# pablode/gatling

Hardware: AMD Instinct MI355X
Metric: Msamples/s (spp x pixels / s) at 8 bounces, 1920x1080 (higher is better)
Workload: dtype f32; 1 GPU; C2: cornell.usda 1920x1080 spp=1024 max-bounces=8 UsdPreviewSurface (diffuse + GGX specular), NEE off; width=1920, height=1080, spp=1024, max_bounces=8, parallelism=single, triangles=46, bvh8_nodes=4

## Files before the change

### gatling_amd/capi.py

```python
from __future__ import annotations

import ctypes as C
import os

import numpy as np

from .scene import P_COUNT, SceneDesc, RenderSettings

_HERE = os.path.dirname(os.path.abspath(__file__))
LIB_PATH = os.path.join(_HERE, "libgatling_gi.so")
if os.environ.get("GATLING_GI_LIB"):
    LIB_PATH = os.path.abspath(os.environ["GATLING_GI_LIB"])

GI_C_OK = 0
AOV_COLOR = 0
FORMAT_INT32, FORMAT_FLOAT32, FORMAT_FLOAT32_VEC4 = 0, 1, 2
OPTION_COUNT_TRAVERSAL, OPTION_KERNEL_TIMERS, OPTION_POOL_SLOTS, OPTION_SAMPLE_BUFFER_MB, OPTION_TRACE_DYNAMIC, OPTION_TWO_LEVEL, OPTION_FUSED_PATH, OPTION_DEVICES = 1, 2, 3, 4, 5, 6, 7, 8
OPTION_SAMPLE_LOOKAHEAD = 10
OPTION_VERTEX_UPDATES = 12
OPTION_VISIBILITY_UPDATES = 11
OPTION_TOPOLOGY_UPDATES = 13
OPTION_RESYNC_REFITS = 14
OPTION_BVH_BUILD = 9

# ... 57 lines not shown
    _fields_ = [("texture", C.c_void_p), ("wrapS", C.c_int32), ("wrapT", C.c_int32), ("channel", C.c_int32),
                ("scale", C.c_float * 4), ("bias", C.c_float * 4)]


class GiCPrimvarData(C.Structure):
    _fields_ = [("name", C.c_char_p), ("type", C.c_int32), ("interpolation", C.c_int32), ("data", C.c_void_p), ("dataSize", C.c_uint64)]



ASSET_OPEN = C.CFUNCTYPE(C.c_void_p, C.c_void_p, C.c_char_p)
ASSET_SIZE = C.CFUNCTYPE(C.c_uint64, C.c_void_p, C.c_void_p)
ASSET_DATA = C.CFUNCTYPE(C.c_void_p, C.c_void_p, C.c_void_p)
ASSET_CLOSE = C.CFUNCTYPE(None, C.c_void_p, C.c_void_p)


class GiCAssetReader(C.Structure):
    _fields_ = [("user", C.c_void_p), ("open", ASSET_OPEN), ("size", ASSET_SIZE), ("data", ASSET_DATA), ("close", ASSET_CLOSE)]


class GiCDecodedImage(C.Structure):
    _fields_ = [("format", C.c_uint32), ("width", C.c_uint32), ("height", C.c_uint32), ("reserved", C.c_uint32), ("pixels", C.c_void_p), ("handle", C.c_void_p)]


IMAGE_LOAD = C.CFUNCTYPE(C.c_int32, C.c_void_p, C.c_char_p, C.c_void_p, C.c_uint64, C.c_int32, C.POINTER(GiCDecodedImage))
IMAGE_RELEASE = C.CFUNCTYPE(None, C.c_void_p, C.POINTER(GiCDecodedImage))
IMAGE_RGBA8_UNORM, IMAGE_RGB16_FLOAT, IMAGE_RGBA16_FLOAT, IMAGE_R32_FLOAT, IMAGE_RGBA32_FLOAT = 1, 2, 3, 4, 5


class GiCImageLoader(C.Structure):
    _fields_ = [("user", C.c_void_p), ("load", IMAGE_LOAD), ("release", IMAGE_RELEASE)]


SYMBOLS = [
    ("giCInitialize", C.c_int, [C.c_int]), ("giCInitializeDevices", C.c_int, [C.POINTER(C.c_int32), C.c_uint32]), ("giCGetDeviceCount", C.c_uint32, []), ("giCGetApiVersion", C.c_uint32, []), ("giCGetDevicePeerAccess", C.c_int32, [C.c_uint32]), ("giCTerminate", None, []), ("giCGetLastError", C.c_char_p, []),
    ("giCCreateMaterial", _P, [_P, C.c_char_p, C.POINTER(GiCMaterialDesc)]), ("giCDestroyMaterial", None, [_P]),
    ("giCCreateMesh", _P, [_P, C.POINTER(GiCMeshDesc)]), ("giCSetMeshTransform", None, [_P, _FP]),
    ("giCSetMeshInstanceTransforms", None, [_P, _U, _FP]), ("giCSetMeshInstanceIds", None, [_P, _U, C.POINTER(C.c_int32)]),
    ("giCSetMeshMaterial", None, [_P, _P]), ("giCSetMeshVisibility", None, [_P, _I]), ("giCSetMeshVertices", C.c_int, [_P, _U, _P]), ("giCDestroyMesh", None, [_P]),
    ("giCRender", C.c_int, [C.POINTER(GiCRenderParams)]),
    ("giCCreateScene", _P, []), ("giCDestroyScene", None, [_P]),
    ("giCCreateSphereLight", _P, [_P]), ("giCDestroySphereLight", None, [_P, _P]), ("giCSetSphereLightPosition", None, [_P, _FP]),
    ("giCSetSphereLightBaseEmission", None, [_P, _FP]), ("giCSetSphereLightRadius", None, [_P, _F, _F, _F]),
    ("giCSetSphereLightDiffuseSpecular", None, [_P, _F, _F]),
    ("giCCreateDistantLight", _P, [_P]), ("giCDestroyDistantLight", None, [_P, _P]), ("giCSetDistantLightDirection", None, [_P, _FP]),
    ("giCSetDistantLightBaseEmission", None, [_P, _FP]), ("giCSetDistantLightAngle", None, [_P, _F]),
    ("giCSetDistantLightDiffuseSpecular", None, [_P, _F, _F]),
    ("giCCreateRectLight", _P, [_P]), ("giCDestroyRectLight", None, [_P, _P]), ("giCSetRectLightOrigin", None, [_P, _FP]),
    ("giCSetRectLightTangents", None, [_P, _FP, _FP]), ("giCSetRectLightBaseEmission", None, [_P, _FP]),
    ("giCSetRectLightDimensions", None, [_P, _F, _F]), ("giCSetRectLightDiffuseSpecular", None, [_P, _F, _F]),
    ("giCCreateDiskLight", _P, [_P]), ("giCDestroyDiskLight", None, [_P, _P]), ("giCSetDiskLightOrigin", None, [_P, _FP]),
    ("giCSetDiskLightTangents", None, [_P, _FP, _FP]), ("giCSetDiskLightBaseEmission", None, [_P, _FP]),
    ("giCSetDiskLightRadius", None, [_P, _F, _F]), ("giCSetDiskLightDiffuseSpecular", None, [_P, _F, _F]),
    ("giCCreateDomeLight", _P, [_P, C.c_char_p]), ("giCDestroyDomeLight", None, [_P]), ("giCSetDomeLightRotation", None, [_P, _FP]),
    ("giCSetDomeLightBaseEmission", None, [_P, _FP]), ("giCSetDomeLightDiffuseSpecular", None, [_P, _F, _F]),
    ("giCSetDomeLightTexture", None, [_P, _P]),
    ("giCCreateTexture", _P, [_P, C.POINTER(GiCTextureDesc)]), ("giCDestroyTexture", None, [_P]),
    ("giCCreateTextureFromFile", _P, [_P, C.c_char_p, _I]),
    ("giCDebugDecodeImage", C.c_int, [C.c_char_p, _I, C.POINTER(C.c_uint32), C.POINTER(C.c_uint32), _FP, C.c_uint64]),
    ("giCRegisterAssetReader", None, [C.POINTER(GiCAssetReader)]), ("giCSetImageLoader", None, [C.POINTER(GiCImageLoader)]),
    ("giCSetMaterialTexture", C.c_int, [_P, _I, C.POINTER(GiCTextureBinding)]),
    ("giCSetMaterialTextureTransform", C.c_int, [_P, _I, _FP]),
    ("giCSetMeshPrimvars", C.c_int, [_P, _U, C.POINTER(GiCPrimvarData)]), ("giCSetMeshInstancerPrimvars", C.c_int, [_P, _U, C.POINTER(GiCPrimvarData)]),
    ("giCSetMaterialPrimvarInput", C.c_int, [_P, _I, C.c_char_p]),
    ("giCCreateRenderBuffer", _P, [_U, _U, _I]), ("giCDestroyRenderBuffer", None, [_P]), ("giCGetRenderBufferMem", _P, [_P]),
    ("giCGetRenderBufferDeviceMem", _P, [_P]), ("giCSetRenderBufferDeviceOnly", None, [_P, _I]),
    ("giCGetRenderStats", C.c_int, [_P, C.POINTER(GiCRenderStats)]), ("giCSetSceneOption", C.c_int, [_P, _I, _I]),
    ("giCGetLookaheadStats", C.c_int, [_P, C.POINTER(GiCLookaheadStats)]),
    ("giCTraceRays", C.c_int, [_P, _U, _FP, _FP, _F, _F, _FP, C.POINTER(C.c_int32)]),
    ("giCDebugEvalBsdf", C.c_int, [C.POINTER(GiCMaterialDesc), _U, _FP, _FP]),
    ("giCDebugShadeClass", C.c_int, [C.POINTER(GiCMaterialDesc)]),
    ("giCDebugCheckSqrt", C.c_int64, [C.c_uint32, C.c_uint64]),
    ("giCDebugValidateBvh", C.c_int, [_FP, _U, C.POINTER(C.c_uint32), C.POINTER(C.c_uint32)]),
    ("giCDebugValidatePartitionedBvh", C.c_int, [_FP, _U, _U, C.POINTER(C.c_uint32), C.POINTER(C.c_uint32)]),
    ("giCDebugValidateSceneBvh", C.c_int, [_P, _U, C.POINTER(C.c_uint32), C.POINTER(C.c_uint32), C.POINTER(C.c_int32), C.POINTER(C.c_uint64)]),
    ("giCDebugTexRuntime", C.c_int, [_FP, _U, _U, _U, _U, _FP, _FP]),
    ("giCDebugEditDirtyFlags", C.c_int32, [_I, _I]), ("giCDebugSceneUpdateCounts", C.c_int, [_P, C.POINTER(C.c_uint64)]),
    ("giCDebugSceneVisibilityUpdateCount", C.c_int, [_P, C.POINTER(C.c_uint64)]), ("giCDebugSceneClassState", C.c_int, [_P, C.POINTER(C.c_uint32)]),
    ("giCDebugSceneVertexUpdateCount", C.c_int, [_P, C.POINTER(C.c_uint64)]), ("giCDebugRefitBvh", C.c_int, [_FP, _FP, _U, C.POINTER(C.c_uint32), C.POINTER(C.c_uint32)]),
    ("giCDebugSceneRefitCheck", C.c_int, [_P, _U, C.POINTER(C.c_uint32)]),
    ("giCDebugSceneTopologyUpdateCount", C.c_int, [_P, C.POINTER(C.c_uint64)]),
    ("giCDebugSceneResyncCount", C.c_int, [_P, C.POINTER(C.c_uint64)]), ("giCDebugGatherShade", C.c_int, [_P, _U, _P, _U]),
    ("giCDebugSceneShadeCheck", C.c_int, [_P, _U, C.POINTER(C.c_uint32)]),
    ("giCDebugPathWalkStats", C.c_int, [_P, C.POINTER(C.c_uint64)]),
    ("giCDebugMissRect", C.c_int, [_FP, C.POINTER(GiCCameraDesc), C.POINTER(GiCRenderSettings), _U, _U, C.POINTER(C.c_uint32)]),
]

_lib = None


def load_library():
    global _lib
    if _lib is None:
        if not os.path.exists(LIB_PATH):
            raise RuntimeError(f"{LIB_PATH} is missing: build it with `python -c 'import __graft_entry__ as g; g.build()'` "
                               "(hipcc --offload-arch=gfx950); there is no CPU fallback")
        L = C.CDLL(LIB_PATH)
        for name, res, args in SYMBOLS:
            fn = getattr(L, name)
            fn.restype = res
            fn.argtypes = args
        _lib = L
    return _lib


def _fp(values):
    arr = (C.c_float * len(values))(*[float(v) for v in values])
    return arr


class GiError(RuntimeError):
    pass


def miss_rect(bounds, camera, rs: "RenderSettings", width: int, height: int):
    L = load_library()
    out = (C.c_uint32 * 4)()
    cam, st = _camera(camera), _settings(rs)
    if L.giCDebugMissRect(_fp(bounds), C.byref(cam), C.byref(st), int(width), int(height), out) != GI_C_OK:
        raise GiError("giCDebugMissRect failed: " + L.giCGetLastError().decode())
    return tuple(int(v) for v in out)


def debug_gather_shade(vertices, faces) -> int:
    from .scene import VERTEX_DTYPE
    L = load_library()
    v = np.ascontiguousarray(vertices, VERTEX_DTYPE)
    f = np.ascontiguousarray(faces, np.uint32).reshape(-1, 3)
    n = L.giCDebugGatherShade(v.ctypes.data, len(v), f.ctypes.data, len(f))
    if n < 0:
        raise GiError("giCDebugGatherShade refused the mesh")
    return int(n)


_initialized = False


def initialize(device: int = 0, devices=None):
    global _initialized
    L = load_library()
    if not _initialized:
        if devices:
            arr = (C.c_int32 * len(devices))(*[int(d) for d in devices])
            rc = L.giCInitializeDevices(arr, len(devices))
        else:
            rc = L.giCInitialize(device)
        if rc != GI_C_OK:
            raise GiError("giCInitialize failed: " + L.giCGetLastError().decode())
        _initialized = True
    return L


def _camera(cam) -> GiCCameraDesc:
    f3 = lambda v: (C.c_float * 3)(*[float(x) for x in v])
    return GiCCameraDesc(f3(cam.position), f3(cam.forward), f3(cam.up), cam.vfov, cam.f_stop, cam.focus_distance,
                         cam.focal_length, cam.clip_start, cam.clip_end, cam.exposure)


def _settings(rs: RenderSettings) -> GiCRenderSettings:
    s = GiCRenderSettings()
    s.clippingPlanes = int(rs.clipping_planes); s.depthOfField = int(rs.depth_of_field)
    s.domeLightCameraVisible = int(rs.dome_light_camera_visible); s.filterImportanceSampling = int(rs.filter_importance_sampling)
    s.frame = float(getattr(rs, "frame", 0.0)); s.jitteredSampling = int(rs.jittered_sampling); s.lightIntensityMultiplier = rs.light_intensity_multiplier
    s.maxBounces = rs.max_bounces; s.maxSampleValue = rs.max_sample_value; s.maxVolumeWalkLength = rs.max_volume_walk_length
    s.mediumStackSize = rs.medium_stack_size; s.metersPerSceneUnit = rs.meters_per_scene_unit
    s.nextEventEstimation = int(rs.next_event_estimation); s.progressiveAccumulation = int(rs.progressive_accumulation)
    s.rrBounceOffset = rs.rr_bounce_offset; s.rrInvMinTermProb = rs.rr_inv_min_term_prob; s.spp = rs.spp; s.time = 0.0
# ... 181 lines not shown
        else:
            m.primvar_inputs.pop(slot, None)
        if self.L.giCSetMaterialPrimvarInput(self.materials[material_index], int(slot), name.encode() if name else None) != GI_C_OK:
            raise GiError("giCSetMaterialPrimvarInput failed: " + self.L.giCGetLastError().decode())

    def _set_primvars(self, fn, h, pvs):
        arr, keep = (GiCPrimvarData * max(len(pvs), 1))(), []
        for k, pv in enumerate(pvs):
            d = np.ascontiguousarray(pv.data, np.int32 if int(pv.type) >= 4 else np.float32).reshape(-1)
            keep.append(d)
            arr[k] = GiCPrimvarData(pv.name.encode(), int(pv.type), int(pv.interpolation), d.ctypes.data, d.nbytes)
        if fn(h, len(pvs), arr) != GI_C_OK:
            raise GiError("giCSetMesh*Primvars failed: " + self.L.giCGetLastError().decode())

    def set_mesh_primvars(self, mesh_index: int, primvars):
        self.desc.meshes[mesh_index].primvars = list(primvars)
        self._set_primvars(self.L.giCSetMeshPrimvars, self.meshes[mesh_index], list(primvars))

    def set_mesh_instancer_primvars(self, mesh_index: int, primvars):
        self.desc.meshes[mesh_index].instancer_primvars = list(primvars)
        self._set_primvars(self.L.giCSetMeshInstancerPrimvars, self.meshes[mesh_index], list(primvars))

    def set_mesh_visibility(self, mesh_index: int, visible: bool):
        self.desc.meshes[mesh_index].visible = bool(visible)
        self.L.giCSetMeshVisibility(self.meshes[mesh_index], int(bool(visible)))

    def set_mesh_vertices(self, mesh_index: int, vertices):
        from .scene import VERTEX_DTYPE
        v = np.ascontiguousarray(vertices, VERTEX_DTYPE)
        if self.L.giCSetMeshVertices(self.meshes[mesh_index], len(v), v.ctypes.data) != GI_C_OK:
            raise GiError("giCSetMeshVertices failed: " + self.L.giCGetLastError().decode())
        self.desc.meshes[mesh_index].vertices = v.copy()

    def vertex_update_count(self) -> int:
        n = C.c_uint64(0)
        if self.L.giCDebugSceneVertexUpdateCount(self.handle, C.byref(n)) != GI_C_OK:
            raise GiError("giCDebugSceneVertexUpdateCount failed")
        return int(n.value)

    def refit_check(self, device: int = 0) -> dict:
        nodes = C.c_uint32(0)
        v = self.L.giCDebugSceneRefitCheck(self.handle, device, C.byref(nodes))
        if v < 0:
            raise GiError("giCDebugSceneRefitCheck failed: " + self.L.giCGetLastError().decode())
        return {"differing": v, "nodes": nodes.value}

    def shade_check(self, device: int = 0) -> int:
        records = C.c_uint32(0)
        v = self.L.giCDebugSceneShadeCheck(self.handle, device, C.byref(records))
        if v < 0:
            raise GiError("giCDebugSceneShadeCheck failed: " + self.L.giCGetLastError().decode())
        return int(v)

    def resync_count(self) -> int:
        n = C.c_uint64(0)
        if self.L.giCDebugSceneResyncCount(self.handle, C.byref(n)) != GI_C_OK:
            raise GiError("giCDebugSceneResyncCount failed")
        return int(n.value)

    def update_counts(self) -> dict:
        c = (C.c_uint64 * 3)()
        if self.L.giCDebugSceneUpdateCounts(self.handle, c) != GI_C_OK:
            raise GiError("giCDebugSceneUpdateCounts failed")
        return {"full": int(c[0]), "transform": int(c[1]), "material": int(c[2])}

    def visibility_update_count(self) -> int:
        n = C.c_uint64(0)
        if self.L.giCDebugSceneVisibilityUpdateCount(self.handle, C.byref(n)) != GI_C_OK:
            raise GiError("giCDebugSceneVisibilityUpdateCount failed")
        return int(n.value)

    def class_state(self) -> dict:
        c = (C.c_uint32 * 5)()
        if self.L.giCDebugSceneClassState(self.handle, c) != GI_C_OK:
            raise GiError("giCDebugSceneClassState failed")
        return {"classMask": int(c[0]), "classTextured": int(c[1]), "shadeClassMask": int(c[2]), "shadeClassTextured": int(c[3]), "hasCutouts": bool(c[4])}

    def path_walk_stats(self) -> dict:
        c = (C.c_uint64 * 18)()
        if self.L.giCDebugPathWalkStats(self.handle, c) != GI_C_OK:
            raise GiError("giCDebugPathWalkStats failed")
        return {"phaseTrips": int(c[0]), "stepTrips": [int(v) for v in c[1:9]], "stepLanes": [int(v) for v in c[9:17]], "fewLaneSteps": int(c[17])}

    def set_option(self, option: int, value: int):
        if self.L.giCSetSceneOption(self.handle, option, value) != GI_C_OK:
            raise GiError("giCSetSceneOption failed")

    def color_buffer(self, width, height):
        key = ("color", width, height)
        if key not in self._buffers:
            rb = self.L.giCCreateRenderBuffer(width, height, FORMAT_FLOAT32_VEC4)
            if not rb:
                raise GiError("giCCreateRenderBuffer failed: " + self.L.giCGetLastError().decode())
            self._buffers[key] = rb
        return self._buffers[key]

    def render(self, settings: RenderSettings, width: int, height: int, rows=None, device_only=False, row_stride=1, copy=True):
        L = self.L
        rb = self.color_buffer(width, height)
        L.giCSetRenderBufferDeviceOnly(rb, int(device_only))
        binding = GiCAovBinding()
        binding.aovId = AOV_COLOR
        clear = np.asarray(settings.clear_color, np.float32)
        C.memmove(binding.clearValue, clear.ctypes.data, 16)
        binding.renderBuffer = rb
        p = GiCRenderParams()
        p.aovBindings = C.pointer(binding)
        p.aovBindingCount = 1
        p.camera = _camera(self.desc.camera)
        p.domeLight = self.dome
        p.renderSettings = _settings(settings)
        p.scene = self.handle
        r0, r1 = rows if rows is not None else (0, height)
        p.rowBegin, p.rowEnd, p.rowStride = r0, r1, row_stride
        if L.giCRender(C.byref(p)) != GI_C_OK:
            raise GiError("giCRender failed: " + L.giCGetLastError().decode())
        if device_only:
            return None
        mem = L.giCGetRenderBufferMem(rb)
        full = np.ctypeslib.as_array(C.cast(mem, C.POINTER(C.c_float)), shape=(height, width, 4))
        return full[r0:r1:row_stride].copy() if copy else full[r0:r1:row_stride]

    AOVS = {"normal": (1, FORMAT_FLOAT32_VEC4), "nee": (2, FORMAT_FLOAT32_VEC4), "barycentrics": (3, FORMAT_FLOAT32_VEC4),
            "texcoords": (4, FORMAT_FLOAT32_VEC4), "bounces": (5, FORMAT_FLOAT32_VEC4), "clockCycles": (6, FORMAT_FLOAT32_VEC4), "opacity": (7, FORMAT_FLOAT32_VEC4),
            "tangents": (8, FORMAT_FLOAT32_VEC4), "bitangents": (9, FORMAT_FLOAT32_VEC4), "thinWalled": (10, FORMAT_FLOAT32_VEC4),
            "objectId": (11, FORMAT_INT32), "depth": (12, FORMAT_FLOAT32), "faceId": (13, FORMAT_INT32), "instanceId": (14, FORMAT_INT32),
            "doubleSided": (15, FORMAT_FLOAT32_VEC4), "albedo": (16, FORMAT_FLOAT32_VEC4)}

    def render_aovs(self, settings: RenderSettings, width: int, height: int, names, clear_values=None, with_color=True, rows=None, row_stride=1):
        L = self.L
        r0, r1 = rows if rows is not None else (0, height)
        bindings = []
        bufs = {}
        if with_color:
            bufs["color"] = (self.color_buffer(width, height), FORMAT_FLOAT32_VEC4, np.asarray(settings.clear_color, np.float32).tobytes(), AOV_COLOR)
        for name in names:
            aid, fmt = self.AOVS[name]
            key = ("aov", name, width, height)
            if key not in self._buffers:
                self._buffers[key] = L.giCCreateRenderBuffer(width, height, fmt)
            cv = (clear_values or {}).get(name, 0)
            if fmt == FORMAT_INT32:
                raw = np.int32(cv).tobytes() + b"\0" * 12
            elif fmt == FORMAT_FLOAT32:
                raw = np.float32(cv).tobytes() + b"\0" * 12
            else:
                cv4 = (list(cv) + [0, 0, 0, 0])[:4] if hasattr(cv, "__len__") else [cv] * 4
                raw = np.asarray(cv4, np.float32).tobytes()
            bufs[name] = (self._buffers[key], fmt, raw, aid)
        arr = (GiCAovBinding * len(bufs))()
        for i, (name, (rb, fmt, raw, aid)) in enumerate(bufs.items()):
            arr[i].aovId = aid
            C.memmove(arr[i].clearValue, raw, 16)
            arr[i].renderBuffer = rb
        p = GiCRenderParams()
        p.aovBindings = C.cast(arr, C.POINTER(GiCAovBinding)); p.aovBindingCount = len(bufs)
        p.camera = _camera(self.desc.camera); p.domeLight = self.dome; p.renderSettings = _settings(settings); p.scene = self.handle
        p.rowBegin, p.rowEnd, p.rowStride = r0, r1, row_stride
        if L.giCRender(C.byref(p)) != GI_C_OK:
            raise GiError("giCRender failed: " + L.giCGetLastError().decode())
        out = {}
        for name, (rb, fmt, raw, aid) in bufs.items():
            mem = L.giCGetRenderBufferMem(rb)
            if fmt == FORMAT_FLOAT32_VEC4:
                a = np.ctypeslib.as_array(C.cast(mem, C.POINTER(C.c_float)), shape=(height, width, 4))
            elif fmt == FORMAT_FLOAT32:
# ... 78 lines not shown
```

### gatling_amd/csrc/gi_debug.cpp

```cpp
#include "gi_host.h"
#include "gi_refit.h"

static int giCTraceRaysImpl(GiCScene* s, uint32_t count, const float* origins, const float* dirs, float tMin, float tMax, float* outTUV, int32_t* outInstPrim);
extern "C" int giCTraceRays(GiCScene* s, uint32_t count, const float* origins, const float* dirs, float tMin, float tMax, float* outTUV, int32_t* outInstPrim)
{
  try { return giCTraceRaysImpl(s, count, origins, dirs, tMin, tMax, outTUV, outInstPrim); }
  catch (const std::exception& e) { setError(std::string("giCTraceRays: ") + e.what()); return -1; }
}
static int giCTraceRaysImpl(GiCScene* s, uint32_t count, const float* origins, const float* dirs, float tMin, float tMax, float* outTUV, int32_t* outInstPrim)
{
  if (!g_ctx.initialized || !s || (count && (!origins || !dirs || !outTUV || !outInstPrim))) { setError("giCTraceRays: bad arguments"); return -1; }
  if (count == 0) return 0;
  std::lock_guard<std::mutex> guard(s->mutex);
  hipStream_t st = g_ctx.stream;
  if (syncSceneGeometry(s) != GI_C_OK) return -1;
  const bool inLds = sceneFitsLds(s->nodeCount, s->triCount);
  const uint32_t blocks = std::min<uint32_t>((count + 255u) / 256u, (uint32_t)g_ctx.cuCount * (inLds ? 3u : 8u));
  if (ensurePathState(s, count, blocks, blocks) != GI_C_OK) return -1;
  const size_t qn = (size_t)s->queueCap * NSHARD;
  std::vector<uint32_t> qslot(qn, 0u); std::vector<F4> qa(qn), qb(qn);
  Counters c{};
  const uint32_t per = (count + NSHARD - 1u) / NSHARD;
  for (uint32_t k = 0; k < NSHARD; k++) { uint32_t lo = k * per; c.count[Q_TRACE_A][k].v = lo < count ? std::min(per, count - lo) : 0u; }
  for (uint32_t i = 0; i < count; i++) {
// ... 412 lines not shown
    case 1: giCDestroyMaterial(matB); matB = nullptr; break;
    case 2: giCSetMeshMaterial(mesh, matB); break;
    case 3: giCSetMaterialPrimvarInput(matA, GI_C_TEX_BASE_COLOR, "k"); break;
    case 4: giCSetMaterialTexture(matA, GI_C_TEX_BASE_COLOR, &binding); break;
    case 5: giCSetMaterialTextureTransform(matA, GI_C_TEX_BASE_COLOR, xf); break;
    case 6: madeTex = giCCreateTexture(s, &td); break;
    case 7: giCDestroyTexture(tex); tex = nullptr; break;
    case 8: giCSetMeshPrimvars(mesh, 1, &pv); break;
    case 9: giCSetMeshInstancerPrimvars(mesh, 1, &pv); break;
    case 10: giCSetMeshTransform(mesh, identity); break;
    case 11: giCSetMeshVisibility(mesh, 0); break;
    case 12: giCSetMeshInstanceIds(mesh, 1, &id); break;
    case 13: madeMesh = giCCreateMesh(s, &meshDesc); break;
    case 14: giCDestroyMesh(mesh); mesh = nullptr; break;
    case 15: giCSetMeshInstanceTransforms(mesh, 0, nullptr); break;
    case 16: if (giCSetMeshVertices(mesh, 3, verts) != GI_C_OK) result = -1; break;
    default: result = -1; break;
  }
  if (result == 0) result = (int32_t)s->dirty;
  if (madeMesh) giCDestroyMesh(madeMesh);
  if (mesh) giCDestroyMesh(mesh);
  if (made) giCDestroyMaterial(made);
  if (matA) giCDestroyMaterial(matA);
  if (matB) giCDestroyMaterial(matB);
  if (madeTex) giCDestroyTexture(madeTex);
  if (tex) giCDestroyTexture(tex);
  return result;
}

extern "C" int giCDebugSceneUpdateCounts(const GiCScene* scene, uint64_t* outCounts)
{
  GiCScene* s = const_cast<GiCScene*>(scene);
  if (!s || !outCounts) { setError("giCDebugSceneUpdateCounts: bad arguments"); return GI_C_ERROR; }
  std::lock_guard<std::mutex> guard(s->mutex);
  outCounts[0] = s->updateCounts[UPDATE_FULL]; outCounts[1] = s->updateCounts[UPDATE_TRANSFORM]; outCounts[2] = s->updateCounts[UPDATE_MATERIAL];
  return GI_C_OK;
}

extern "C" int giCDebugSceneVisibilityUpdateCount(const GiCScene* scene, uint64_t* outCount)
{
  GiCScene* s = const_cast<GiCScene*>(scene);
  if (!s || !outCount) { setError("giCDebugSceneVisibilityUpdateCount: bad arguments"); return GI_C_ERROR; }
  std::lock_guard<std::mutex> guard(s->mutex);
  *outCount = s->updateCounts[UPDATE_VISIBILITY];
  return GI_C_OK;
}

extern "C" int giCDebugSceneVertexUpdateCount(const GiCScene* scene, uint64_t* outCount)
{
  GiCScene* s = const_cast<GiCScene*>(scene);
  if (!s || !outCount) { setError("giCDebugSceneVertexUpdateCount: bad arguments"); return GI_C_ERROR; }
  std::lock_guard<std::mutex> guard(s->mutex);
  *outCount = s->updateCounts[UPDATE_VERTEX];
  return GI_C_OK;
}

extern "C" int giCDebugSceneTopologyUpdateCount(const GiCScene* scene, uint64_t* outCount)
{
  GiCScene* s = const_cast<GiCScene*>(scene);
  if (!s || !outCount) { setError("giCDebugSceneTopologyUpdateCount: bad arguments"); return GI_C_ERROR; }
  std::lock_guard<std::mutex> guard(s->mutex);
  *outCount = s->updateCounts[UPDATE_TOPOLOGY];
  return GI_C_OK;
}

extern "C" int giCDebugSceneResyncCount(const GiCScene* scene, uint64_t* outCount)
{
  GiCScene* s = const_cast<GiCScene*>(scene);
  if (!s || !outCount) { setError("giCDebugSceneResyncCount: bad arguments"); return GI_C_ERROR; }
  std::lock_guard<std::mutex> guard(s->mutex);
  *outCount = s->resyncCount;
  return GI_C_OK;
}

extern "C" int giCDebugPathWalkStats(const GiCScene* scene, uint64_t* out)
{
  GiCScene* s = const_cast<GiCScene*>(scene);
  if (!s || !out) { setError("giCDebugPathWalkStats: bad arguments"); return GI_C_ERROR; }
  std::lock_guard<std::mutex> guard(s->mutex);
  for (int k = 0; k < 18; k++) out[k] = s->pathWalkStats[k];
  return GI_C_OK;
}

extern "C" int giCDebugSceneClassState(const GiCScene* scene, uint32_t* out)
{
  GiCScene* s = const_cast<GiCScene*>(scene);
  if (!s || !out) { setError("giCDebugSceneClassState: bad arguments"); return GI_C_ERROR; }
  std::lock_guard<std::mutex> guard(s->mutex);
  out[0] = s->classMask; out[1] = s->classTextured; out[2] = s->shadeClassMask; out[3] = s->shadeClassTextured; out[4] = s->hasCutouts ? 1u : 0u;
  return GI_C_OK;
}
```

### gatling_amd/csrc/gi_host.h

```cpp

#pragma once

#pragma GCC visibility push(default)
#include "../../include/gi_c.h"
#pragma GCC visibility pop


#include <algorithm>
#include <atomic>
#include <chrono>
#include <cmath>
#include <cstdio>
#include <cstdlib>
#include <cstring>
#include <memory>
#include <condition_variable>
#include <functional>
#include <mutex>
#include <string>
#include <thread>
#include <vector>

#include "bvh8.h"
#include "gi_kernels.h"
// ... 133 lines not shown
template <typename Rec, typename Handle>
struct DenseStore {
  std::vector<Rec> recs;
  std::vector<Handle*> owners;
  uint32_t add(Handle* h, const Rec& r) { recs.push_back(r); owners.push_back(h); return (uint32_t)recs.size() - 1u; }
  void remove(uint32_t idx);
};

struct GiCSphereLight { GiCScene* scene; uint32_t index; };
struct GiCDistantLight { GiCScene* scene; uint32_t index; };
struct GiCRectLight { GiCScene* scene; uint32_t index; };
struct GiCDiskLight { GiCScene* scene; uint32_t index; };
struct GiCDomeLight { GiCScene* scene; std::string filePath; GiCTexture* texture = nullptr; bool ownsTexture = false; float rotation[4] = {0, 0, 0, 1};
    float baseEmission[3] = {1, 1, 1}; float diffuse = 1.0f, specular = 1.0f; };

template <typename Rec, typename Handle>
void DenseStore<Rec, Handle>::remove(uint32_t idx)
{
  uint32_t last = (uint32_t)recs.size() - 1u;
  if (idx != last) { recs[idx] = recs[last]; owners[idx] = owners[last]; owners[idx]->index = idx; }
  recs.pop_back(); owners.pop_back();
}

struct GiCRenderBuffer {
  uint32_t width, height, stride;
  size_t size;
  void* deviceMem = nullptr;
  void* hostMem = nullptr;
  bool deviceOnly = false;
  bool scratch = false;
  std::vector<void*> replicaMem;
  void* stageMem = nullptr;
};

struct LookaheadKey {
  FrameUniforms U;
  SceneView view;
  uint64_t generation;
};
struct Lookahead {
  bool valid = false;
  uint32_t calls = 0, served = 0, firstOffset = 0;
  uint32_t pixelMajor = 0;
  LookaheadKey key{};
  uint32_t traced = 0;
  uint64_t windowsTraced = 0, callsServed = 0, windowsDiscarded = 0, samplesUnused = 0;
  void drop()
  {
    if (valid && served < calls) { windowsDiscarded++; samplesUnused += (uint64_t)(calls - served) * key.U.spp; }
    valid = false; calls = served = 0;
  }
};

struct SceneDevice {
  uint32_t slot = 0;
  DeviceBuffer<MeshRec> dMeshes; DeviceBuffer<float> dSceneData;
  std::vector<DeviceBuffer<float>*> dTexels; DeviceBuffer<TextureRec> dTextures;
  std::vector<uint64_t> dTexelSerial;
  DeviceBuffer<Node8> dNodes; DeviceBuffer<TriRec> dTris; DeviceBuffer<InstanceRec> dInstances;
  DeviceBuffer<FVertex> dVerts; DeviceBuffer<MaterialRec> dMaterials; DeviceBuffer<int32_t> dTriFaceId; DeviceBuffer<TriShade> dTriShade;
      DeviceBuffer<F4> dTriGeomNormal;
  DeviceBuffer<SphereLightRec> dSphere; DeviceBuffer<DistantLightRec> dDistant; DeviceBuffer<RectLightRec> dRect; DeviceBuffer<DiskLightRec> dDisk;
  DeviceBuffer<LightFrame> dRectFrames, dDiskFrames;
  DeviceBuffer<Node8> dTlasNodes, dBlasNodes; DeviceBuffer<uint32_t> dTlasItems, dFlatOfOrig; DeviceBuffer<BlasTri> dBlasTris; DeviceBuffer<InstTrav> dInstTrav;
  DeviceBuffer<Slot> slots;
  DeviceBuffer<float> media;
  DeviceBuffer<F4> scratchColor; DeviceBuffer<unsigned long long> neeKey;
  DeviceBuffer<uint32_t> pathSegments;
  DeviceBuffer<F4> sampleBuf;
  Lookahead lookahead;
  DeviceBuffer<F4> accum;
  DeviceBuffer<uint32_t> qSlot[Q_COUNT];
  DeviceBuffer<F4> qA[Q_COUNT], qB[Q_COUNT], qC[Q_COUNT];
  DeviceBuffer<FreshRec> qFresh[2];
  uint32_t queueCap = 0;
  DeviceBuffer<Counters> dCounters;
  Counters* hCounters = nullptr;
  uint64_t memTotalMb = 0;
  static constexpr uint32_t POLL_RING = 4, POLL_LAG = 2;
  PaddedCounter* hPoll = nullptr; hipEvent_t pollEvent[POLL_RING] = {};
  hipEvent_t evShade = nullptr, evShadow = nullptr;
  GiCRenderStats stats{};
  uint64_t pathWalkStats[18] = {};
  std::vector<hipEvent_t> eventPool;
  template <typename Fn> void forEachPathBuffer(Fn&& fn)
  {
    fn(slots); fn(media); fn(sampleBuf);
    for (uint32_t q = 0; q < Q_COUNT; q++) { fn(qSlot[q]); fn(qA[q]); fn(qB[q]); fn(qC[q]); }
    fn(qFresh[0]); fn(qFresh[1]);
  }
  uint64_t pathStateBytes() { uint64_t n = 0; forEachPathBuffer([&](auto& b) { n += b.bytes(); }); return n; }
  void releasePathState() { forEachPathBuffer([](auto& b) { b.release(); }); queueCap = 0; lookahead.drop(); }
  void releaseAll();
};

struct TwoLevelHost { std::vector<Node8> tlasNodes, blasNodes; std::vector<uint32_t> tlasItems; std::vector<BlasTri> blasTris; std::vector<InstTrav> instTrav;
    };
struct MeshBuild { const GiCMesh* m; uint32_t vertexOffset, matFlags, instFirst, instCount, triFirst; uint32_t meshIdx; std::vector<int32_t> faceIdAov;
    uint32_t shadeBase = 0;
    bool hidden = false; uint32_t idBase = 0; };
struct InstPart { uint32_t meshBuild, instInMesh; uint32_t triFirst, nf; uint32_t nodeOff, nodeCount, nodeCap, depth; float box[6];
    uint32_t activeTris = 0; std::vector<uint32_t> levelStart; };
struct SceneHost {
  std::vector<FVertex> verts; std::vector<InstanceRec> instances; std::vector<MaterialRec> mats; std::vector<MeshRec> meshRecs; std::vector<float> sceneData;
  Bvh8 bvh; std::vector<int32_t> triFaceId; std::vector<uint32_t> flatOfOrig; TwoLevelHost two;
  std::vector<MeshBuild> meshBuilds;
  std::vector<F4> triGeomNormal;
  std::vector<TriShade> triShade; bool shadePacked = false;
  bool partitioned = false; std::vector<InstPart> parts; uint32_t topCap = 0;
  bool deviceBuilt = false;
  bool hostTreeDropped = false;
  bool reordered = false;
};

enum : uint32_t { UPDATE_FULL = 0, UPDATE_TRANSFORM = 1, UPDATE_MATERIAL = 2, UPDATE_VISIBILITY = 3, UPDATE_VERTEX = 4, UPDATE_TOPOLOGY = 5 };
struct GiCScene : SceneDevice {
  std::mutex mutex;
  uint32_t dirty = DIRTY_ALL;
  std::vector<GiCMesh*> meshes;
  std::vector<GiCMaterial*> materials;
  std::vector<GiCTexture*> textures;
  uint64_t nextTextureSerial = 1;
  DenseStore<SphereLightRec, GiCSphereLight> sphereLights;
  DenseStore<DistantLightRec, GiCDistantLight> distantLights;
  DenseStore<RectLightRec, GiCRectLight> rectLights;
  DenseStore<DiskLightRec, GiCDiskLight> diskLights;
  uint32_t lightCounts[4] = {0, 0, 0, 0};
  uint32_t sampleOffset = 0;
  bool haveOldParams = false;
  GiCCameraDesc oldCamera{};
  GiCRenderSettings oldSettings{};
  uint8_t oldClear[GI_C_MAX_AOV_COMP_SIZE] = {0};
  uint32_t oldRowBegin = 0, oldRowEnd = 0, oldRowStride = 1;
  GiCDomeLight* oldDome = nullptr;
  float oldDomeEmission[3] = {0, 0, 0};
  uint32_t nodeCount = 0, triCount = 0, bvhDepth = 0;
  float bounds[6] = {0, 0, 0, 0, 0, 0}; bool boundsValid = false;
  int optBvhBuild = 0;
  bool twoLevel = false; int optTwoLevel = -1;
  bool hasCutouts = false;
  bool shadePacked = false;
  uint32_t classMask = 0;
  uint32_t classTextured = 0;
  uint32_t shadeClassMask = 0, shadeClassTextured = 0;
  std::unique_ptr<SceneHost> host;
  std::vector<std::unique_ptr<SceneDevice>> replicas;
  bool countTraversal = false, kernelTimers = false;
  uint32_t kernelTimerStride = 1;
  uint64_t optPoolSlots = 0, optSampleBufferMb = 0;
  int32_t optFusedPath = -1;
  int32_t optTraceDyn = -1;
  std::atomic<int32_t> shadowOrder{-1};
       uint64_t shadowOrderRays[2] = {0, 0},
      shadowOrderSteps[2] = {0, 0};
  int32_t optDevices = 0;
  uint32_t lastRenderDevices = 0;
  int32_t optLookahead = 0;
  uint64_t generation = 0;
  uint64_t updateCounts[6] = {0, 0, 0, 0, 0, 0};
  int32_t optVisibilityUpdates = 0;
  int32_t optVertexUpdates = 0;
  bool rebuildDue = true;
  int32_t optTopologyUpdates = 0;
  bool topologyDue = false;
  int32_t optResyncRefits = 0; uint64_t resyncCount = 0;
  std::vector<GiCMesh*> retiredMeshes;
// ... 23 lines not shown
```

### gatling_amd/csrc/gi_kernels.h

```cpp
#pragma once

#include <type_traits>
#include <hip/hip_runtime.h>

#include "gi_types.h"

namespace gi {

template <class F>
auto dispatchBools(F&& f) { return f(); }
template <class F, class... Bools>
auto dispatchBools(F&& f, bool b, Bools... rest)
{
  return b ? dispatchBools([&](auto... cs) { return f(std::true_type{}, cs...); }, rest...)
           : dispatchBools([&](auto... cs) { return f(std::false_type{}, cs...); }, rest...);
}

void launchInit(hipStream_t s, const PathState& st, const QueueSet& qs, Counters* cnt, uint32_t n, bool resetStats);
void launchRaygen(hipStream_t s, uint32_t blocks, const FrameUniforms& U, const PathState& st, const QueueSet& qs, Counters* cnt, uint32_t par, F4* sampleBuf);
void launchAccumulate(hipStream_t s, const FrameUniforms& U, const F4* sampleBuf, F4* accum, F4* colorOut, bool firstBatch, bool lastBatch);
void launchFoldWindow(hipStream_t s, const FrameUniforms& U, const F4* sampleBuf, F4* colorOut, uint32_t windowSamples, uint32_t first, bool pixelMajor);
bool traceBlockSync(const SceneView& sc);
bool sceneFitsLds(size_t nodeCount, size_t triCount);
uint32_t traceLdsBytes(uint32_t stackEntries, uint32_t ldsNodes, uint32_t ldsTris);
uint32_t blocksPerCuByLds(uint32_t dynamicBytes, uint32_t staticBytes);
uint32_t traceStaticLdsBytes();
void traceLdsLayout(const SceneView& sc, uint32_t& ldsNodes, uint32_t& ldsTris, uint32_t& bytes);
void launchTrace(hipStream_t s, uint32_t blocks, bool anyHit, bool count, const SceneView& sc, const PathState& st, const QueueSet& qs, Counters* cnt,
                 uint32_t qIn, uint32_t qMiss, uint32_t dynRefill, uint32_t routeBlocks, const FrameUniforms& U, F4* sampleBuf);
void launchRoute(hipStream_t s, uint32_t blocks, const SceneView& sc, const PathState& st, const QueueSet& qs, Counters* cnt, uint32_t qIn, uint32_t qMiss,
    const FrameUniforms& U,
                 F4* sampleBuf);
constexpr uint32_t APPEND_ITEMS_MAX = 4u;
constexpr uint32_t TRACE_DYN_SLOT_ORDER = 0x200u;
void launchShade(hipStream_t s, uint32_t blocks, uint32_t klass, bool textured ,
    bool volume , const FrameUniforms& U, const SceneView& sc, const PathState& st, const QueueSet& qs, Counters* cnt, uint32_t par);

bool pathKernelSupports(const SceneView& sc);
int launchPath(hipStream_t s, uint32_t cuCount, uint32_t classMask, bool textured, bool count, uint32_t chunk, uint32_t walkCarry, const FrameUniforms& U,
               const SceneView& sc, const PathState& st, Counters* cnt, F4* sampleBuf);
constexpr long WALK_CARRY_DEFAULT = 8;

void launchAov(hipStream_t s, const FrameUniforms& U, const SceneView& sc, const AovTargets& A);
void launchResolveNee(hipStream_t s, const FrameUniforms& U, const unsigned long long* key, F4* aov, uint32_t pixelCount);
void launchZeroClosest(hipStream_t s, Counters* cnt, uint32_t par);
void launchPatchMatFlags(hipStream_t s, TriRec* tris, uint32_t triCount, const InstanceRec* instances, uint32_t instanceCount, const uint32_t* wordOfMesh,
    uint32_t meshCount);
struct VisPatch { int32_t idDelta; uint32_t action; };
constexpr uint32_t VIS_KEEP = 0u, VIS_HIDE = 1u, VIS_SHOW = 2u;
void launchPatchVisibility(hipStream_t s, TriRec* tris, uint32_t triCount, const InstanceRec* instances, uint32_t instanceCount, const VisPatch* patchOfInstance,
    const TriShade* triShade, uint32_t shadeCount);
void launchPlacePart(hipStream_t s, const Node8* partNodes, uint32_t partNodeCount, Node8* nodes, uint32_t nodeOff, TriRec* tris, uint32_t triFirst, uint32_t nf,
    uint32_t idAdd);
struct RefitRange { uint32_t threadBase, nodeFirst; };
void launchRefitTris(hipStream_t s, TriRec* tris, uint32_t triCount, const InstanceRec* instances, uint32_t instanceCount, const uint32_t* editedOfInstance,
    const TriShade* triShade, uint32_t shadeCount);
bool gatherShadeRangeOk(uint32_t shadeCount, uint32_t first, uint32_t count);
bool launchGatherShade(hipStream_t s, TriShade* triShade, uint32_t shadeCount, uint32_t first, uint32_t count, const FVertex* verts, uint32_t vertCount);
void launchRefitLevel(hipStream_t s, Node8* nodes, uint32_t nodeCount, float* boxes, const RefitRange* ranges, uint32_t rangeCount, uint32_t threads,
    const TriRec* tris, uint32_t triCount, const InstanceRec* instances, uint32_t instanceCount, const TriShade* triShade, uint32_t shadeCount);
void launchSpin(hipStream_t s, unsigned long long ns);
void launchDebugBsdf(hipStream_t s, const MaterialRec* mat, uint32_t shadeClass, uint32_t count, const float* in, float* out);
void launchDebugSqrt(hipStream_t s, uint32_t first, unsigned long long count, unsigned long long* mismatches);
void launchDebugTex(hipStream_t s, const float* texels, uint32_t w, uint32_t h, uint32_t d, uint32_t count, const float* queries, float* out);

}
```

### gatling_amd/csrc/gi_kernels.hip

```cpp

#include <type_traits>
#include <hip/hip_runtime.h>

#include "gi_device_math.h"
#include "gi_kernels.h"
#include "gi_types.h"
#include "gi_queues.h"
#include "gi_traversal.h"
#include "gi_shading.h"
#include "gi_stages.h"

namespace gi {

__global__ void k_init(PathState st, QueueSet qs, Counters* cnt, uint32_t n, uint32_t resetStats)
{
  uint32_t i = blockIdx.x * blockDim.x + threadIdx.x;
  const uint32_t per = (n + NSHARD - 1u) / NSHARD;
  if (i < Q_COUNT * NSHARD) {
    const uint32_t q = i / NSHARD, sdx = i % NSHARD;
    uint32_t c = 0;
    if (q == Q_REGEN_A) { const uint32_t lo = sdx * per; c = lo < n ? ((n - lo) < per ? (n - lo) : per) : 0u; }
    cnt->count[q][sdx].v = c;
  }
  if (i == 0) {
    if (resetStats) cnt->overflow = 0u;
    cnt->workBase[0].v = 0; cnt->workBase[1].v = 0; for (uint32_t k = 0; k < NCURSOR; k++) { cnt->cursor[0][k].v = 0; cnt->cursor[1][k].v = 0; }
    if (resetStats) { cnt->shadowOrderRays[0] = 0; cnt->shadowOrderRays[1] = 0;
        for (int k = 0; k < 16; k++) { cnt->shadowOrderSteps[0][k].v = 0; cnt->shadowOrderSteps[1][k].v = 0; }
                      cnt->segments = 0; cnt->shadowRays = 0; cnt->nodesVisited = 0; cnt->trisTested = 0; cnt->shadowNodesVisited = 0;
                          cnt->shadowTrisTested = 0;
                      for (int k = 0; k < 4; k++) { cnt->phaseCycles[k] = 0; cnt->phaseLanes[k] = 0; } cnt->phaseTrips = 0;
                      for (int k = 0; k < 8; k++) { cnt->walkStepLanes[k] = 0; cnt->walkStepTrips[k] = 0; } cnt->walkFewLaneSteps = 0;
                          for (int k = 0; k < 8; k++) cnt->dynStats[k] = 0; }
  }
  for (; i < n; i += gridDim.x * blockDim.x) qs.slot[Q_REGEN_A][(i / per) * qs.cap + (i % per)] = i | REGEN_FRESH;
}

constexpr int RAYGEN_ITEMS = 2; static_assert(RAYGEN_ITEMS <= (int)APPEND_ITEMS_MAX, "shardCapacity's slack");
__global__ __launch_bounds__(64) void k_zero_closest(Counters* cnt, uint32_t par) { zero_closest_counters(cnt, par); }
__global__ __launch_bounds__(64) void k_spin(unsigned long long ns, uint32_t* sink)
{
  const unsigned long long t0 = wall_clock64();
  while ((wall_clock64() - t0) * 10ull < ns) { }
  if (sink && threadIdx.x == 0xffffu) *sink = 0u;
}
__global__ __launch_bounds__(BLOCK) void k_raygen(FrameUniforms U, PathState st, QueueSet qs, Counters* cnt, uint32_t par, F4* __restrict__ sampleBuf)
{
  __shared__ AppendScratch<2> sh;
  const uint32_t qIn = Q_REGEN_A + par, qOut = Q_TRACE_A + par, qAgain = Q_REGEN_A + (par ^ 1u);
  const bool boundsRetire = (U.flags & FLAG_BOUNDS_RETIRE) != 0u;
  QueueReader rd; reader_init(rd, cnt, qIn, qs.cap);
  const uint32_t n = rd.pre[NSHARD];
  const uint32_t workBase = cnt->workBase[par].v;
  uint32_t nRetired = 0u;
  if (blockIdx.x == 0) {
    zero_next_counters(cnt, par, !boundsRetire, (U.flags & FLAG_TWO_STREAM) != 0u);
    if (threadIdx.x == 0) { const uint32_t left = U.workTotal - workBase; cnt->workBase[par ^ 1u].v = workBase + (n < left ? n : left); }
  }
  const uint32_t stride = gridDim.x * BLOCK * RAYGEN_ITEMS;
  const uint32_t qid[2] = {qOut, qAgain};
  uint32_t trip = 0;
  for (uint32_t base = blockIdx.x * BLOCK * RAYGEN_ITEMS; base < n; base += stride, trip++) {
    uint32_t which[RAYGEN_ITEMS], idx[RAYGEN_ITEMS], slotOf[RAYGEN_ITEMS]; FreshRec freshOf[RAYGEN_ITEMS];
    V3 originOf[RAYGEN_ITEMS], dirOf[RAYGEN_ITEMS]; float tMinOf[RAYGEN_ITEMS], tMaxOf[RAYGEN_ITEMS];
    uint32_t entryOf[RAYGEN_ITEMS];
#pragma unroll
    for (int k = 0; k < RAYGEN_ITEMS; k++) {
      const uint32_t i = base + (uint32_t)k * BLOCK + threadIdx.x;
      entryOf[k] = i < n ? qs.slot[qIn][reader_index(rd, i)] : 0u;
    }
#pragma unroll
    for (int k = 0; k < RAYGEN_ITEMS; k++) {
      const uint32_t i = base + (uint32_t)k * BLOCK + threadIdx.x;
      bool more = false; uint32_t slot = 0, rng = 0u; FreshRec fresh{0u, 0u};
      V3 origin = v3(0.0f, 0.0f, 0.0f), dir = origin; float tMin = 0.0f, tMax = GI_FLT_MAX;
      if (i < n) {
        const uint32_t entry = entryOf[k];
        slot = entry & ~(REGEN_MISSED | REGEN_FRESH);
        Slot* S = &st.slots[slot];
        F4 id = F4{0.0f, 0.0f, 0.0f, 0.0f};
        if (!(entry & REGEN_FRESH)) id = ld4(&S->id);
        if (f2u(id.z) != 0u) {
          F4 r = ld4(&S->rad);
          V3 rad = v3(r.x, r.y, r.z);
          if (entry & REGEN_MISSED) {
            F4 tb = ld4(&S->thr);
            rad = rad + v3(tb.x, tb.y, tb.z) * v3(U.background);
            if (st.neeKey && (f2u(tb.w) & 0x00000fffu) == 0u) nee_aov_record(st, slot, false);
          }
          if (st.bouncesAov && U.batchFirstSample + f2u(id.y) == U.spp - 1u) {
            const uint32_t bounces = ((f2u(S->thr.w) + ((entry & REGEN_MISSED) ? 1u : 0u)) & 0x00000fffu), maxB = U.maxBounces < 0x00000fffu
                ? U.maxBounces : 0x00000fffu;
            const V3 c = gi_colormap_inferno((float)bounces / (float)maxB);
            F4* dst = &st.bouncesAov[tile_to_image_pixel(U, f2u(id.x))];
            dst->x = c.x; dst->y = c.y; dst->z = c.z;
          }
          if (st.pathSegments) atomicAdd(&st.pathSegments[f2u(id.x)], (f2u(S->thr.w) + ((entry & REGEN_MISSED) ? 1u : 0u)) & 0x00000fffu);
          float mv = fmax2(rad.x, fmax2(rad.y, rad.z));
          if (mv > U.maxSampleValue) rad = rad * (U.maxSampleValue / mv);
          st4(&sampleBuf[sample_record(U, f2u(id.x), f2u(id.y))], fmax2(0.0f, rad.x), fmax2(0.0f, rad.y), fmax2(0.0f, rad.z), 0.0f);
        }
        const uint32_t w = workBase + i;
        more = (i < U.workTotal - workBase) && (w < U.workTotal);
        if (more) {
          uint32_t pixelLocal, sLocal; work_item(U, w, pixelLocal, sLocal);
          const uint32_t pixelIndex = tile_to_image_pixel(U, pixelLocal);
          const uint32_t sampleIndex = U.sampleOffset + U.batchFirstSample + sLocal;
          make_camera_ray(U, pixelIndex, sampleIndex, origin, dir, tMin, tMax, rng);
          fresh.rng = rng; fresh.work = w;
          if (!(U.flags & FLAG_DEFER_SLOT)) slot_begin_path(S, rng, pixelLocal, sLocal);
        }
      }
      bool again = false;
      if (boundsRetire && more && ray_misses_bounds(U, origin, dir, tMin, tMax)) { retire_fresh_miss(U, fresh, sampleBuf); more = false; again = true;
          nRetired++; }
// ... 203 lines not shown
```

### gatling_amd/csrc/gi_path.hip

```cpp

#include <hip/hip_runtime.h>

#define GI_LEAN_SQRT 1
#include "gi_device_math.h"
#include "gi_kernels.h"
#include "gi_types.h"
#include "gi_queues.h"
#include "gi_traversal.h"
#include "gi_shading.h"
#include "gi_stages.h"

namespace gi {

constexpr uint32_t PRE_FIELDS = 10;
constexpr uint32_t PATH_STACK_MAX = 8;

constexpr int PATH_WAVES = 4;
template <uint32_t KLASS, bool TEXTURED, bool NEE, bool CUTOUT, bool COUNT, uint32_t PATH_STACK>
__global__ __launch_bounds__(TRACE_BLOCK) __attribute__((amdgpu_waves_per_eu(PATH_WAVES, 8))) void k_path(FrameUniforms U, SceneView sc, PathState st,
    Counters* cnt, F4* __restrict__ sampleBuf, uint32_t ldsNodes, uint32_t ldsTris, uint32_t chunk, uint32_t walkCarry)
{
  constexpr bool CARRY = !NEE;
  const StagedScene S = stage_scene<PATH_STACK>(sc, ldsNodes, ldsTris);
  __shared__ WaveTri s_wave[TRACE_BLOCK / 64];
  WaveTri& W = s_wave[threadIdx.x >> 6];

  const uint32_t lane = __lane_id();
  const unsigned long long below = (1ull << lane) - 1ull;
  V3 thr = v3(0.0f, 0.0f, 0.0f), rad = thr, ro = thr, rdv = v3(0.0f, 0.0f, 1.0f);
  float tMin = 0.0f, tMax = 0.0f;
  uint32_t bitfield = 0u, rng = 0u, rec = 0u;
  bool alive = false, tAlive = false;
  uint32_t chunkNext = 0u, chunkEnd = 0u; bool exhausted = false;
  uint32_t nSeg = 0u, nShadow = 0u;
  TraceCounters tc{0u, 0u}, tcs{0u, 0u};
  uint2 overflow[1];
  RayTrav R; R.G = make_uint2(0u, 0u); R.sp = 0u;
  __shared__ uint32_t s_pre[TRACE_BLOCK / 64][PRE_FIELDS][128];
  GI_LDS uint32_t (*pre)[128] = (GI_LDS uint32_t (*)[128])&s_pre[threadIdx.x >> 6][0][0];
  uint32_t preHead = 0u, preTail = 0u;
  const bool boundsRetire = (U.flags & FLAG_BOUNDS_RETIRE) != 0u;

  unsigned long long pc[4] = {0ull, 0ull, 0ull, 0ull}, pl[4] = {0ull, 0ull, 0ull, 0ull}, trips = 0ull, tPrev = COUNT ? __builtin_readcyclecounter() : 0ull;
  uint32_t whLanes[8] = {0u, 0u, 0u, 0u, 0u, 0u, 0u, 0u}, whTrips[8] = {0u, 0u, 0u, 0u, 0u, 0u, 0u, 0u};
  uint32_t whFew = 0u;
  auto phase = [&](int k,
      unsigned long long lanes) { if (COUNT) { const unsigned long long t = __builtin_readcyclecounter(); pc[k] += t - tPrev; tPrev = t; pl[k] += lanes; } };
  for (;;) {
    __atomic_signal_fence(__ATOMIC_SEQ_CST);
    unsigned long long idle = __ballot(!alive);
    const uint32_t nIdle = (uint32_t)__popcll(idle);
    if (nIdle) {
      while (preTail - preHead < 64u && !exhausted) {
        if (chunkNext == chunkEnd) {
          uint32_t b = 0u;
          if (lane == 0u) b = atomicAdd(&cnt->cursor[0][0].v, chunk);
          b = (uint32_t)__shfl((int)b, 0);
          if (b >= U.workTotal) { exhausted = true; break; }
          chunkNext = b; chunkEnd = (U.workTotal - b) < chunk ? U.workTotal : b + chunk;
        }
        const uint32_t avail = chunkEnd - chunkNext, take = avail < 64u ? avail : 64u;
        uint32_t nKept = 0u;
        if (lane < take) {
          const uint32_t w = chunkNext + lane;
          const uint32_t sl = w / U.activeCount, a = w - sl * U.activeCount;
          const uint32_t ar = a / U.activeWidth, row = U.rectTy0 + ar, px = U.rectX0 + (a - ar * U.activeWidth);
          const uint32_t rec = sl * U.pixelCount + (row * U.imageWidth + px);
          const uint32_t py = U.rowBegin + row * U.rowStride;
          V3 o, d; float t0, t1; uint32_t r;
          make_camera_ray_at(U, px, py, py * U.imageWidth + px, U.sampleOffset + U.batchFirstSample + sl, o, d, t0, t1, r);
          float lo[3] = {U.sceneLo[0], U.sceneLo[1], U.sceneLo[2]}, hi[3] = {U.sceneHi[0], U.sceneHi[1], U.sceneHi[2]};
          asm volatile("" : "+s"(lo[0]), "+s"(lo[1]), "+s"(lo[2]), "+s"(hi[0]), "+s"(hi[1]), "+s"(hi[2]));
          const bool keep = !(boundsRetire && ray_misses_box(lo, hi, o, d, t0, t1));
          const unsigned long long kept = __ballot(keep);
          nKept = (uint32_t)__popcll(kept);
          if (keep) {
            const uint32_t slot = (preTail + (uint32_t)__popcll(kept & below)) & 127u;
            pre[0][slot] = f2u(o.x); pre[1][slot] = f2u(o.y); pre[2][slot] = f2u(o.z); pre[3][slot] = f2u(d.x); pre[4][slot] = f2u(d.y); pre[5][slot] = f2u(d.z);
            pre[6][slot] = f2u(t0); pre[7][slot] = f2u(t1); pre[8][slot] = r; pre[9][slot] = rec;
          } else {
            float bg[3] = {U.background[0], U.background[1], U.background[2]}, maxv = U.maxSampleValue;
            asm volatile("" : "+s"(bg[0]), "+s"(bg[1]), "+s"(bg[2]), "+s"(maxv));
            V3 c = v3(0.0f, 0.0f, 0.0f) + v3(1.0f, 1.0f, 1.0f) * v3(bg[0], bg[1], bg[2]);
            const float mv = fmax2(c.x, fmax2(c.y, c.z));
            if (mv > maxv) c = c * (maxv / mv);
            st4(&sampleBuf[rec], fmax2(0.0f, c.x), fmax2(0.0f, c.y), fmax2(0.0f, c.z), 0.0f);
            nSeg++;
          }
        }
        chunkNext += take; preTail += (uint32_t)__builtin_amdgcn_readfirstlane((int)nKept);
      }
      __atomic_signal_fence(__ATOMIC_SEQ_CST);
      const uint32_t have = preTail - preHead, take = nIdle < have ? nIdle : have;
      const uint32_t rank = (uint32_t)__popcll(idle & below);
      if (!alive && rank < take) {
        const uint32_t slot = (preHead + rank) & 127u;
        ro = v3(u2f(pre[0][slot]), u2f(pre[1][slot]), u2f(pre[2][slot])); rdv = v3(u2f(pre[3][slot]), u2f(pre[4][slot]), u2f(pre[5][slot]));
        tMin = u2f(pre[6][slot]); tMax = u2f(pre[7][slot]); rng = pre[8][slot];
        rec = pre[9][slot];
        thr = v3(1.0f, 1.0f, 1.0f); rad = v3(0.0f, 0.0f, 0.0f); bitfield = 0u;
        alive = true;
      }
      preHead += take;
    }
    if (!__ballot(alive)) break;
    phase(0, nIdle); trips++;

    {
      const bool carried = CARRY && tAlive;
      const uint2 G = R.G; const uint32_t sp = R.sp;
      trav_init(R, ro, rdv, tMin, alive ? tMax : 0.0f);
      if (carried) { R.G = G; R.sp = sp; R.tBest = u2f(wt_best_t(W, lane)); }
      else wave_ray_begin(W, R.tBest);
    }
    tAlive = alive;
    if (CARRY) {
      unsigned long long walking = __ballot(tAlive);
      const uint32_t stop = (uint32_t)__popcll(walking) > walkCarry ? walkCarry : 0u;
      uint32_t step = 0u;
      while ((uint32_t)__popcll(walking) > stop) {
        if (COUNT) {
          const uint32_t n = (uint32_t)__popcll(walking);
          whLanes[step] += n; whTrips[step]++; step = step < 7u ? step + 1u : 7u;
          if (n < 8u) whFew++;
        }
        if (wave_step<false, COUNT, PATH_STACK, false, STAGED_ALL, CUTOUT>(R, tAlive, W, sc, S, overflow, tc, rng)) tAlive = false;
        walking = __ballot(tAlive);
      }
    } else {
      while (__ballot(tAlive)) {
        if (wave_step<false, COUNT, PATH_STACK, false, STAGED_ALL, CUTOUT>(R, tAlive, W, sc, S, overflow, tc, rng)) tAlive = false;
      }
    }
    const bool walked = CARRY ? alive && !tAlive : alive;
    bool ended = false;
    ShadeIO io; io.shadow = false; io.shadowFirst = false; io.cont = false;
    phase(1, (unsigned long long)__popcll(__ballot(walked)));
    if (walked) {
      nSeg++;
      wave_ray_end(W, R);
      if (R.found) {
        io.throughput = thr; io.radiance = rad; io.bitfield = bitfield; io.rng = rng;
        const F4 h = F4{R.tBest, R.bestU, R.bestV, u2f(R.bestTri)}, rd = F4{rdv.x, rdv.y, rdv.z, 0.0f};
        shade_segment<KLASS, TEXTURED, false, NEE>(U, sc, nullptr, h, rd, io);
        thr = io.throughput; rad = io.radiance; bitfield = io.bitfield; rng = io.rng;
        if (NEE && st.neeKey && io.shadowFirst && !io.shadow) nee_aov_record_px(st, rec % U.pixelCount, rec / U.pixelCount, false);
        ended = !io.cont;
      } else {
        rad = rad + thr * v3(U.background);
        if (st.neeKey && (bitfield & 0x00000fffu) == 0u) nee_aov_record_px(st, rec % U.pixelCount, rec / U.pixelCount, false);
        bitfield++;
        ended = true;
      }
    }
    phase(2, (unsigned long long)__popcll(__ballot(walked && R.found)));

    if (NEE) {
      bool sAlive = alive && io.shadow;
      if (__ballot(sAlive)) {
        trav_init(R, io.no, io.sdir, 0.01f, sAlive ? io.ld : 0.0f);
        wave_ray_begin(W, R.tBest);
        const bool traced = sAlive;
        while (__ballot(sAlive)) {
          if (wave_step<true, COUNT, PATH_STACK, false, STAGED_ALL, CUTOUT>(R, sAlive, W, sc, S, overflow, tcs, io.rngShadow)) sAlive = false;
        }
        if (traced) {
          nShadow++;
          if (!R.found) rad = rad + io.nee;
          if (st.neeKey && io.shadowFirst) nee_aov_record_px(st, rec % U.pixelCount, rec / U.pixelCount, R.found);
        }
      }
    }

    if (walked) {
      if (!ended) { ro = io.no; rdv = io.k2; tMin = 0.0f; tMax = io.tMaxNext; }
      else {
        const uint32_t bounces = bitfield & 0x00000fffu;
        if (st.bouncesAov && U.batchFirstSample + rec / U.pixelCount == U.spp - 1u) {
          const uint32_t maxB = U.maxBounces < 0x00000fffu ? U.maxBounces : 0x00000fffu;
          const V3 c = gi_colormap_inferno((float)bounces / (float)maxB);
          F4* dst = &st.bouncesAov[tile_to_image_pixel(U, rec % U.pixelCount)];
          dst->x = c.x; dst->y = c.y; dst->z = c.z;
        }
        if (st.pathSegments) atomicAdd(&st.pathSegments[rec % U.pixelCount], bounces);
        const V3 c = finish_sample(U, rad);
        st4(&sampleBuf[rec], c.x, c.y, c.z, 0.0f);
        alive = false;
      }
    }
    phase(3, (unsigned long long)__popcll(__ballot(ended)));
  }

  if (COUNT
      && lane == 0u) { for (int k = 0; k < 4; k++) { atomicAdd(&cnt->phaseCycles[k], pc[k]); atomicAdd(&cnt->phaseLanes[k], pl[k]);
      } atomicAdd(&cnt->phaseTrips, trips);
      for (int k = 0; k < 8; k++) { atomicAdd(&cnt->walkStepLanes[k], (unsigned long long)whLanes[k]); atomicAdd(&cnt->walkStepTrips[k], (unsigned long long)whTrips[k]); }
      atomicAdd(&cnt->walkFewLaneSteps, (unsigned long long)whFew); }
  unsigned long long a = nSeg, b = nShadow, c = tc.nodes, d = tc.tris, e = tcs.nodes, f = tcs.tris;
  for (int off = 32; off > 0; off >>= 1) {
    a += __shfl_down(a, off); b += __shfl_down(b, off);
    if (COUNT) { c += __shfl_down(c, off); d += __shfl_down(d, off); e += __shfl_down(e, off); f += __shfl_down(f, off); }
  }
  if (lane == 0u) {
    atomicAdd(&cnt->segments, a);
    if (NEE) atomicAdd(&cnt->shadowRays, b);
    if (COUNT) { atomicAdd(&cnt->nodesVisited, c); atomicAdd(&cnt->trisTested, d); atomicAdd(&cnt->shadowNodesVisited, e); atomicAdd(&cnt->shadowTrisTested, f);
        }
  }
}

bool pathKernelSupports(const SceneView& sc)
{
  return sc.triCount > 0u && sceneFitsLds(sc.nodeCount, sc.triCount) && sc.bvhDepth <= PATH_STACK_MAX && sc.mediumStackSize == 0u
      && sc.domeTexture == 0u && !sc.twoLevel
         && !sc.shadePacked;
}

using PathKernel = void (*)(FrameUniforms, SceneView, PathState, Counters*, F4*, uint32_t, uint32_t, uint32_t, uint32_t);
template <uint32_t STACK>
static PathKernel pickPathKernel(uint32_t classMask, bool textured, bool nee, bool cutout, bool count)
{
  const bool hot = (classMask == 1u || classMask == 2u || classMask == 4u) && !textured && !cutout && !count;
  return dispatchBools([&](auto neeC) -> PathKernel {
    constexpr bool NEE = decltype(neeC)::value;
    if (hot) {
      if (classMask == 1u) return k_path<0u, false, NEE, false, false, STACK>;
      if (classMask == 2u) return k_path<1u, false, NEE, false, false, STACK>;
      return k_path<2u, false, NEE, false, false, STACK>;
    }
    return dispatchBools([](auto countC) -> PathKernel { return k_path<KLASS_DYNAMIC, true, NEE, true, decltype(countC)::value, STACK>; }, count);
  }, nee);
}

int launchPath(hipStream_t s, uint32_t cuCount, uint32_t classMask, bool textured, bool count, uint32_t chunk, uint32_t walkCarry, const FrameUniforms& U,
               const SceneView& sc, const PathState& st, Counters* cnt, F4* sampleBuf)
{
  if (U.workTotal == 0u) return 0;
  const uint32_t ldsNodes = sc.nodeCount, ldsTris = sc.triCount;
  const uint32_t stack = sc.bvhDepth <= 4u ? 4u : 8u;
  const uint32_t bytes = traceLdsBytes(stack, ldsNodes, ldsTris);
  const bool neeOn = (U.flags & FLAG_NEE) != 0u;
  PathKernel k = stack == 4u
      ? pickPathKernel<4u>(classMask, textured, neeOn, sc.hasCutouts != 0u, count) : pickPathKernel<8u>(classMask, textured, neeOn, sc.hasCutouts != 0u, count);
  int perCu = 2;
  hipFuncAttributes fa{};
  if (hipFuncGetAttributes(&fa, reinterpret_cast<const void*>(k)) == hipSuccess && fa.numRegs > 0) {
    const uint32_t regs = ((uint32_t)fa.numRegs + 7u) & ~7u, byRegs = 512u / regs;
    const uint32_t byLds = blocksPerCuByLds(bytes, (uint32_t)fa.sharedSizeBytes);
    perCu = (int)(byRegs < byLds ? byRegs : byLds);
    if (perCu > 8) perCu = 8;
    if (perCu < 1) perCu = 1;
  }
  const uint64_t chunks = ((uint64_t)U.workTotal + chunk - 1u) / chunk;
  uint64_t blocks = (uint64_t)cuCount * (uint64_t)perCu;
  const uint64_t needed = (chunks + (TRACE_BLOCK / 64u) - 1u) / (TRACE_BLOCK / 64u);
  if (blocks > needed) blocks = needed;
  if (blocks == 0u) blocks = 1u;
  hipLaunchKernelGGL(k, dim3((uint32_t)blocks), dim3(TRACE_BLOCK), bytes, s, U, sc, st, cnt, sampleBuf, ldsNodes, ldsTris, chunk, walkCarry);
  return perCu;
}

__global__ void k_debug_sqrt(uint32_t first, unsigned long long count, unsigned long long* mismatches)
{
  unsigned long long bad = 0ull;
  for (unsigned long long i = blockIdx.x * (unsigned long long)blockDim.x + threadIdx.x; i < count; i += (unsigned long long)gridDim.x * blockDim.x) {
    const float x = u2f(first + (uint32_t)i);
    const float a = gi_sqrt(x), b = sqrtf(x);
    if (f2u(a) != f2u(b) && !(a != a && b != b)) bad++;
  }
  if (bad) atomicAdd(mismatches, bad);
}

void launchDebugSqrt(hipStream_t s, uint32_t first, unsigned long long count, unsigned long long* mismatches)
{
  hipLaunchKernelGGL(k_debug_sqrt, dim3(4096), dim3(256), 0, s, first, count, mismatches);
}

}
```

### gatling_amd/csrc/gi_render.cpp

```cpp
#include "gi_host.h"
#include "gi_miss_rect.h"

bool settingsEqual(const GiCRenderSettings& a, const GiCRenderSettings& b) { return memcmp(&a, &b, sizeof(a)) == 0; }

SceneView makeView(GiCScene* s, SceneDevice& D)
{
  SceneView v{};
  v.textures = D.dTextures.ptr; v.meshes = D.dMeshes.ptr; v.sceneData = D.dSceneData.ptr;
  v.nodes = D.dNodes.ptr; v.tris = D.dTris.ptr; v.instances = D.dInstances.ptr;
  v.verts = D.dVerts.ptr; v.triShade = D.dTriShade.ptr; v.triGeomNormal = D.dTriGeomNormal.ptr; v.shadePacked = s->shadePacked ? 1u : 0u;
      v.materials = D.dMaterials.ptr;
      v.sphereLights = D.dSphere.ptr; v.distantLights = D.dDistant.ptr;
  v.tlasNodes = D.dTlasNodes.ptr; v.tlasItems = D.dTlasItems.ptr; v.blasNodes = D.dBlasNodes.ptr; v.blasTris = D.dBlasTris.ptr; v.instTrav = D.dInstTrav.ptr;
      v.flatOfOrig = D.dFlatOfOrig.ptr; v.twoLevel = s->twoLevel ? 1u : 0u;
  v.rectLights = D.dRect.ptr; v.diskLights = D.dDisk.ptr; v.rectFrames = D.dRectFrames.ptr; v.diskFrames = D.dDiskFrames.ptr; v.triFaceId = D.dTriFaceId.ptr;
      v.nodeCount = s->nodeCount; v.triCount = s->triCount;
      v.bvhDepth = s->bvhDepth; v.hasCutouts = s->hasCutouts ? 1u : 0u;
  return v;
}
SceneView makeView(GiCScene* s) { return makeView(s, *s); }

uint32_t traceDynRefill(const GiCScene* s)
{
  long r = s->optTraceDyn;
// ... 263 lines not shown
    sizeGrids(p, in);
  }
  p.mediaStride = rs.mediumStackSize ? rs.mediumStackSize * MEDIUM_FLOATS + 4u : 0u;
  p.pinned = optionSet("pool_slots") || s->optPoolSlots || optionSet("sample_buffer_mb") || s->optSampleBufferMb;
  if (!p.pinned) while (planBytes(p, pixels) > (availMb << 20) - std::min<uint64_t>(availMb << 19, 512ull << 20) && shrinkPlan(p, pixels)) sizeGrids(p, in);
  return p;
}

static int allocatePathPlan(GiCScene* s, SceneDevice& D, const GiCRenderSettings& rs, uint64_t samples, const SceneView& view, const PlanInputs& in,
                            PathPlan& plan)
{
  size_t memFree = 0, memTotal = 0; (void)hipMemGetInfo(&memFree, &memTotal);
  if (optionSet("assume_free_mb")) memFree = (size_t)optionValue("assume_free_mb", 0) << 20;
  if (!D.memTotalMb) D.memTotalMb = std::max<uint64_t>(1, (uint64_t)(memTotal >> 20));
  plan = planPathMemory(s, rs, samples, view, in, memFree, D.pathStateBytes(), D.memTotalMb);
  for (int attempt = 0;; attempt++) {
    int rc = plan.fused ? GI_C_OK : ensurePathState(&D, plan.slots, plan.wideBlocks, plan.traceBlocks);
    if (rc == GI_C_OK) rc = D.sampleBuf.alloc(in.pixels * plan.batchSamples);
    if (rc == GI_C_OK) rc = D.accum.alloc(in.pixels);
    if (rc == GI_C_OK && plan.mediaStride) rc = D.media.alloc(plan.slots * plan.mediaStride);
    if (rc == GI_C_OK) { if (attempt > 0) t_lastError.clear(); return GI_C_OK; }
    if (rc != GI_C_OUT_OF_MEMORY_INTERNAL) return GI_C_ERROR;
    D.releasePathState();
    if (attempt >= 40 || !shrinkPlan(plan, in.pixels)) {
      setError("giCRender: out of device memory even with the smallest sample buffer and path pool");
      return GI_C_ERROR;
    }
    sizeGrids(plan, in);
  }
}

struct StageTimers {
  enum Kind { RAYGEN = 0, TRACE = 1, SHADE = 2, SHADOW = 3 };
  struct IterRow { size_t evEnd; uint64_t traced, hits, shadow, ended, cont; };
  SceneDevice& D;
  bool on; uint32_t stride;
  bool iterLog;
  bool sampling = false;
  size_t ev = 0; std::vector<int> evKind;
  std::vector<IterRow> iterRows;
  uint64_t totalIters = 0, sampledIters = 0;

  StageTimers(const GiCScene* s, SceneDevice& d) : D(d), on(s->kernelTimers), stride(std::max(1u, s->kernelTimerStride)),
      iterLog(on && stride == 1u && getenv("GATLING_ITER_LOG") && atoi(getenv("GATLING_ITER_LOG")) != 0) {}
  void beginIteration(bool always = false) { sampling = on && (always || (totalIters % stride) == 0u); if (sampling) sampledIters++; }
  template <typename Fn> void timed(hipStream_t stream, int kind, Fn&& fn)
  {
    if (!sampling) { fn(); return; }
    (void)hipEventRecord(poolEvent(&D, ev), stream); fn(); (void)hipEventRecord(poolEvent(&D, ev + 1), stream);
    ev += 2; evKind.push_back(kind);
  }
  void finish(GiCRenderStats& S) const;
};

void StageTimers::finish(GiCRenderStats& S) const
{
  S.traceMs = S.shadeMs = S.raygenMs = S.shadowMs = 0.0;
  if (!on) return;
  auto elapsed = [&](size_t k) { float ms = 0.0f; (void)hipEventElapsedTime(&ms, D.eventPool[2 * k], D.eventPool[2 * k + 1]); return ms; };
  for (size_t k = 0; k < evKind.size(); k++) {
    const float ms = elapsed(k);
    if (evKind[k] == RAYGEN) S.raygenMs += ms; else if (evKind[k] == TRACE) S.traceMs += ms; else if (evKind[k] == SHADE) S.shadeMs += ms;
    else S.shadowMs += ms;
  }
  size_t k = 0;
  for (size_t r = 0; r < iterRows.size(); r++) {
    const IterRow& row = iterRows[r];
    double ms4[4] = {0.0, 0.0, 0.0, 0.0};
    for (; 2 * k < row.evEnd && k < evKind.size(); k++) ms4[evKind[k]] += elapsed(k);
    fprintf(stderr, "[gatling_gi] iter %3zu: rays %9llu hits %9llu shadow %9llu ended %9llu continuing %9llu | raygen %7.3f trace+route %7.3f shade %7.3f "
                    "shadow %7.3f ms\n", r,
            (unsigned long long)row.traced, (unsigned long long)row.hits, (unsigned long long)row.shadow, (unsigned long long)row.ended,
            (unsigned long long)row.cont, ms4[0], ms4[1], ms4[2], ms4[3]);
  }
  const double scale = sampledIters ? (double)totalIters / (double)sampledIters : 1.0;
  S.raygenMs *= scale; S.traceMs *= scale; S.shadeMs *= scale; S.shadowMs *= scale;
}

struct Schedule {
  bool twoStreamOk = false;
  long twoStreamDelay = 0;
  uint32_t dynRefill = 8u;
  uint32_t walkCarry = 0u;
  int32_t shadowOrderNow = -1;
};
struct Frame {
  GiCScene* s; SceneDevice& D; const DevCtx& ctx; const RenderJob& job; const GiCRenderSettings& rs;
  hipStream_t st;
  size_t pixels;
  StageTimers tm;
  FrameUniforms U{}; SceneView view{};
  PathPlan plan; PathState ps{}; QueueSet qs{}; Schedule sch;
  F4* colorOut = nullptr;
  uint32_t numBatches = 0;
  uint32_t iters = 0, traceLaunches = 0;
  double tStart = 0.0;
  uint32_t windowCalls = 0;
  bool served = false;
  uint64_t skippedSegments = 0;
};

static int bindPathAovs(Frame& f, const BoundAovs& A)
{
  SceneDevice& D = f.D;
  f.ps = PathState{D.slots.ptr, D.media.ptr, f.plan.mediaStride, nullptr, 0u, nullptr};
  if (A.nee && f.rs.nextEventEstimation) {
    if (D.neeKey.alloc(f.pixels)) return GI_C_ERROR;
    HIP_TRY(hipMemsetAsync(D.neeKey.ptr, 0, f.pixels * sizeof(unsigned long long), f.st));
    f.ps.neeKey = D.neeKey.ptr;
  }
  if (A.bounces) f.ps.bouncesAov = reinterpret_cast<F4*>(rbMem(A.bounces, D.slot));
  if (A.clock) {
    if (D.pathSegments.alloc(f.pixels)) return GI_C_ERROR;
    HIP_TRY(hipMemsetAsync(D.pathSegments.ptr, 0, f.pixels * sizeof(uint32_t), f.st));
    f.ps.pathSegments = D.pathSegments.ptr;
  }
  return GI_C_OK;
}

static Schedule scheduleFrame(Frame& f)
{
  const GiCScene* s = f.s; const GiCRenderSettings& rs = f.rs; FrameUniforms& U = f.U;
  const bool fused = f.plan.fused;
  if (!fused && optionValue("work_order", WORK_ORDER_PIXEL_MAJOR_DEFAULT ? 1 : 0) != 0) U.flags |= FLAG_PIXEL_MAJOR;
  if (!fused && optionValue("defer_slot", 1) != 0 && !f.ps.neeKey && !f.ps.bouncesAov && !f.ps.pathSegments) U.flags |= FLAG_DEFER_SLOT;
  if ((U.flags & FLAG_DEFER_SLOT) && !traceBlockSync(f.view) && !f.view.twoLevel && f.view.domeTexture == 0u && rs.mediumStackSize == 0u && !s->countTraversal
      && s->boundsValid && optionValue("bounds_retire", 1) != 0) {
    U.flags |= FLAG_BOUNDS_RETIRE;
    for (int a = 0; a < 3; a++) { U.sceneLo[a] = s->bounds[a]; U.sceneHi[a] = s->bounds[3 + a]; }
  }
  if (fused && s->boundsValid && optionValue("bounds_retire", 1) != 0 && !s->countTraversal && !f.ps.neeKey && !f.ps.bouncesAov && !f.ps.pathSegments) {
    U.flags |= FLAG_BOUNDS_RETIRE;
    for (int a = 0; a < 3; a++) { U.sceneLo[a] = s->bounds[a]; U.sceneHi[a] = s->bounds[3 + a]; }
  }
  if (fused) {
    U.rectX0 = 0u; U.rectX1 = U.imageWidth; U.rectTy0 = 0u; U.rectTy1 = f.job.tileRows;
    if ((U.flags & FLAG_BOUNDS_RETIRE) && U.maxBounces > 0u && f.windowCalls < 2u && optionValue("miss_rect", 1) != 0) {
      const MissRect r = computeMissRect(U.sceneLo, U.sceneHi, U, U.imageWidth, U.imageHeight);
      uint32_t ty0, ty1; missRectTileRows(r, U.rowBegin, U.rowStride, f.job.tileRows, ty0, ty1);
      if (r.empty() || ty1 <= ty0) { U.rectX0 = U.rectX1 = U.rectTy0 = U.rectTy1 = 0u; }
      else { U.rectX0 = r.x0; U.rectX1 = r.x1; U.rectTy0 = ty0; U.rectTy1 = ty1; }
    }
    U.activeWidth = U.rectX1 - U.rectX0; U.activeCount = U.activeWidth * (U.rectTy1 - U.rectTy0);
    if (U.activeCount < U.pixelCount) U.flags |= FLAG_MISS_RECT;
  }
  Schedule sch;
  sch.walkCarry = s->countTraversal && !optionSet("walk_carry") ? 0u : (uint32_t)std::min(std::max(optionValue("walk_carry", WALK_CARRY_DEFAULT), 0L), 63L);
  sch.dynRefill = traceDynRefill(s);
  sch.shadowOrderNow = optionSet("shadow_order") ? (int32_t)optionValue("shadow_order", -1) : s->shadowOrder.load();
  sch.twoStreamOk = rs.nextEventEstimation != 0 && rs.mediumStackSize == 0u && f.view.domeTexture == 0u && optionValue("two_stream", 1) != 0
                    && f.ctx.stream2 != nullptr;
  sch.twoStreamDelay = optionValue("two_stream_delay", 0);
  return sch;
}
static bool scheduleBatch(Frame& f, uint64_t rounds)
{
  const GiCScene* s = f.s; FrameUniforms& U = f.U;
  const long mergeOpt = optionValue("merge_shade_variants", -1);
  const bool thinBatch = rounds == 1 && U.workTotal <= (8u << 20);
  if ((mergeOpt < 0 ? thinBatch : mergeOpt != 0) && (s->shadeClassMask & (1u << SHADE_CLASS_OPBR_BASE)) && (s->shadeClassMask & 4u)) {
    U.flags |= FLAG_MERGE_SHADE_VARIANTS;
  } else U.flags &= ~FLAG_MERGE_SHADE_VARIANTS;
  const bool two = f.sch.twoStreamOk && rounds == 1 && !f.tm.iterLog;
  if (two) U.flags |= FLAG_TWO_STREAM; else U.flags &= ~FLAG_TWO_STREAM;
  return two;
}

static void accumulateBatch(Frame& f, uint32_t batch)
{
  if (f.windowCalls >= 2u) {
    launchFoldWindow(f.st, f.U, f.D.sampleBuf.ptr, f.colorOut, f.U.batchSamples, 0u, (f.U.flags & FLAG_PIXEL_MAJOR) != 0u);
    return;
  }
  launchAccumulate(f.st, f.U, f.D.sampleBuf.ptr, f.D.accum.ptr, f.colorOut, batch == 0, batch + 1 == f.numBatches);
}

static int runFusedBatch(Frame& f, uint32_t batch)
{
  const GiCScene* s = f.s; SceneDevice& D = f.D; const FrameUniforms& U = f.U;
  uint32_t chunk = 2048u;
  const uint64_t waves = (uint64_t)f.ctx.cuCount * 16u;
  chunk = (uint32_t)std::min<uint64_t>(chunk, std::max<uint64_t>(64u, ((uint64_t)U.workTotal / (waves * 16u)) & ~63ull));
  f.tm.beginIteration(true);
  f.tm.timed(f.st, StageTimers::TRACE, [&] {
    launchPath(f.st, (uint32_t)f.ctx.cuCount, s->classMask, s->classTextured != 0u, s->countTraversal, chunk, f.sch.walkCarry, U, f.view, f.ps,
               D.dCounters.ptr, D.sampleBuf.ptr);
  });
  f.iters++; f.tm.totalIters++; f.traceLaunches++;
  accumulateBatch(f, batch);
  return GI_C_OK;
}

static int runZeroBounceBatch(Frame& f, uint32_t batch)
{
  HIP_TRY(hipMemsetAsync(f.D.sampleBuf.ptr, 0, f.pixels * f.U.batchSamples * sizeof(F4), f.st));
  accumulateBatch(f, batch);
  return GI_C_OK;
}

static int runWavefrontBatch(Frame& f, uint32_t batch, uint32_t poolNow)
{
  GiCScene* s = f.s; SceneDevice& D = f.D; FrameUniforms& U = f.U; StageTimers& tm = f.tm;
  const GiCRenderSettings& rs = f.rs; const PathPlan& plan = f.plan; const Schedule& sch = f.sch;
  hipStream_t st = f.st, st2 = f.ctx.stream2;
  const uint64_t rounds = ((uint64_t)U.workTotal + poolNow - 1) / poolNow;
  const uint64_t maxIters = (rounds + 2) * (std::max(1u, U.maxBounces) + 1) + 8;
  const bool two = scheduleBatch(f, rounds);
  const bool nee = rs.nextEventEstimation != 0;
  bool shadowInFlight = false;
  struct JoinShadow {
    hipStream_t st2; const bool& inFlight;
    ~JoinShadow() { if (inFlight) (void)hipStreamSynchronize(st2); }
  } joinOnError{st2, shadowInFlight};
  auto joinShadow = [&]() -> hipError_t {
    if (!shadowInFlight) return hipSuccess;
    const hipError_t e = hipStreamWaitEvent(st, D.evShadow, 0);
    if (e == hipSuccess) shadowInFlight = false;
    return e;
  };
  for (uint64_t it = 0; it < maxIters; it++) {
    const uint32_t par = (uint32_t)(it & 1u);
    tm.beginIteration();
    auto raygen = [&] { tm.timed(st, StageTimers::RAYGEN, [&] { launchRaygen(st, plan.wideBlocks, U, f.ps, f.qs, D.dCounters.ptr, par, D.sampleBuf.ptr); }); };
    if (two) launchZeroClosest(st, D.dCounters.ptr, par);
    if (!two || it == 0) raygen();
    else if (rounds == 1 && it == (uint64_t)std::max(1u, U.maxBounces)) { HIP_TRY(joinShadow()); raygen(); }
    if (rounds == 1 && it == (uint64_t)std::max(1u, U.maxBounces) && rs.mediumStackSize == 0u) { tm.totalIters++; break; }
    if (it >= rounds) {
      constexpr uint32_t R = SceneDevice::POLL_RING, LAG = SceneDevice::POLL_LAG;
      constexpr size_t snapshot = (size_t)Q_COUNT * NSHARD;
      HIP_TRY(hipMemcpyAsync(D.hPoll + (it % R) * snapshot, D.dCounters.ptr, sizeof(PaddedCounter) * snapshot, hipMemcpyDeviceToHost, st));
      HIP_TRY(hipEventRecord(D.pollEvent[it % R], st));
      if (it >= rounds + LAG) {
        const uint64_t j = it - LAG;
        HIP_TRY(hipEventSynchronize(D.pollEvent[j % R]));
        const PaddedCounter* snap = D.hPoll + (j % R) * snapshot + (size_t)(Q_TRACE_A + (uint32_t)(j & 1u)) * NSHARD;
        const PaddedCounter* again = D.hPoll + (j % R) * snapshot + (size_t)(Q_REGEN_A + (uint32_t)((j & 1u) ^ 1u)) * NSHARD;
        uint32_t pending = 0; for (uint32_t k = 0; k < NSHARD; k++) pending += snap[k].v + again[k].v;
        if (pending == 0) { tm.totalIters++; break; }
      }
    }
    if (two && sch.twoStreamDelay == 1) launchSpin(st, 300000ull);
    tm.timed(st, StageTimers::TRACE, [&] {
      launchTrace(st, plan.traceBlocks, false, s->countTraversal, f.view, f.ps, f.qs, D.dCounters.ptr, Q_TRACE_A + par, Q_REGEN_A + (par ^ 1u), sch.dynRefill,
                  plan.wideBlocks, U, D.sampleBuf.ptr);
    });
    f.traceLaunches++;
    if (two && it > 0) { HIP_TRY(joinShadow()); raygen(); }
    uint32_t shadeMask = s->shadeClassMask | ((rs.mediumStackSize != 0u && (s->shadeClassMask & (1u << SHADE_CLASS_OPBR_BASE))) ? 4u : 0u);
    if (U.flags & FLAG_MERGE_SHADE_VARIANTS) shadeMask = (shadeMask & ~(1u << SHADE_CLASS_OPBR_BASE)) | ((shadeMask >> SHADE_CLASS_OPBR_BASE) & 1u) << 2;
    for (uint32_t klass = 0; klass < MAT_CLASS_COUNT; klass++) {
      if (!(shadeMask & (1u << klass))) continue;
      tm.timed(st, StageTimers::SHADE, [&] {
        launchShade(st, plan.wideBlocks, klass, (s->shadeClassTextured & (1u << klass)) != 0u, rs.mediumStackSize != 0u, U, f.view, f.ps, f.qs, D.dCounters.ptr,
                    par);
      });
    }
    if (nee) {
      const int32_t order = sch.shadowOrderNow >= 0 ? sch.shadowOrderNow : (int32_t)(tm.totalIters & 1u);
      hipStream_t on = st;
      if (two) {
        HIP_TRY(hipEventRecord(D.evShade, st)); HIP_TRY(hipStreamWaitEvent(st2, D.evShade, 0));
        if (sch.twoStreamDelay == 2) launchSpin(st2, 300000ull);
        on = st2;
      }
      tm.timed(on, StageTimers::SHADOW, [&] {
        launchTrace(on, plan.traceBlocks, true, s->countTraversal, f.view, f.ps, f.qs, D.dCounters.ptr, Q_SHADOW, Q_SHADOW,
                    sch.dynRefill | (order ? TRACE_DYN_SLOT_ORDER : 0u), plan.wideBlocks, U, D.sampleBuf.ptr);
      });
      if (two) { shadowInFlight = true; HIP_TRY(hipEventRecord(D.evShadow, st2)); }
    }
    if (tm.iterLog) {
      HIP_TRY(hipMemcpyAsync(D.hCounters, D.dCounters.ptr, sizeof(PaddedCounter) * Q_COUNT * NSHARD, hipMemcpyDeviceToHost, st));
      HIP_TRY(hipStreamSynchronize(st));
      auto total = [&](uint32_t q) { uint64_t n = 0; for (uint32_t k = 0; k < NSHARD; k++) n += D.hCounters->count[q][k].v; return n; };
      uint64_t hits = 0; for (uint32_t c = 0; c < MAT_CLASS_COUNT; c++) hits += total(Q_HIT + c);
      tm.iterRows.push_back({tm.ev, total(Q_TRACE_A + par), hits, total(Q_SHADOW), total(Q_REGEN_A + (par ^ 1u)), total(Q_TRACE_A + (par ^ 1u))});
    }
    f.iters++; tm.totalIters++;
  }
  HIP_TRY(joinShadow());
  accumulateBatch(f, batch);
  return GI_C_OK;
}

static int finishPathAovs(Frame& f, const BoundAovs& A)
{
  SceneDevice& D = f.D; const RenderJob& job = f.job; hipStream_t st = f.st;
  const size_t pixels = f.pixels; const uint32_t width = job.width, rowBegin = job.rowBegin, rowStride = job.rowStride;
  if (A.nee && f.ps.neeKey) launchResolveNee(st, f.U, D.neeKey.ptr, reinterpret_cast<F4*>(rbMem(A.nee, D.slot)), (uint32_t)pixels);
  if (GiCRenderBuffer* clockRb = A.clock) {
    std::vector<uint32_t> counts(pixels);
    HIP_TRY(hipMemcpyAsync(counts.data(), D.pathSegments.ptr, pixels * sizeof(uint32_t), hipMemcpyDeviceToHost, st));
    HIP_TRY(hipStreamSynchronize(st));
    float maxValue = 0.0f;
    for (uint32_t c : counts) maxValue = std::max(maxValue, (float)c);
    float* img = reinterpret_cast<float*>(clockRb->hostMem);
    for (size_t p = 0; p < pixels; p++) {
      const size_t y = rowBegin + (p / width) * rowStride, x = p % width;
      float* o = img + (y * width + x) * 4;
      if (maxValue > 0.0f) {
        const int idx = std::min((int)(((float)counts[p] / maxValue) * 255.0), 255);
        turboColormap((float)idx / 255.0f, o);
        o[3] = 255.0f;
      } else { o[0] = (float)counts[p]; o[1] = 0.0f; o[2] = 0.0f; }
    }
    HIP_TRY(hipMemcpyAsync(rbMem(clockRb, D.slot), clockRb->hostMem, clockRb->size, hipMemcpyHostToDevice, st));
  }
  if (A.bounces && f.U.maxBounces == 0u) {
    float* img = reinterpret_cast<float*>(A.bounces->hostMem);
    for (size_t p = 0; p < pixels; p++) { float* o = img + ((rowBegin + (p / width) * rowStride) * width + p % width) * 4; o[0] = o[1] = o[2] = NAN; }
    HIP_TRY(hipMemcpyAsync(rbMem(A.bounces, D.slot), A.bounces->hostMem, A.bounces->size, hipMemcpyHostToDevice, st));
  }
  for (GiCRenderBuffer* rb : {A.nee, A.bounces}) {
    if (!rb || rb->deviceOnly || !job.readback) continue;
    HIP_TRY(copyTileRows(rb, rb->stride, job, D.slot, st));
  }
  return GI_C_OK;
}

static int runAovPass(Frame& f, const BoundAovs& A)
{
  launchAov(f.st, f.U, f.view, A.targets);
  if (hipGetLastError() != hipSuccess) { setError("k_aov launch failed"); return GI_C_ERROR; }
  for (GiCRenderBuffer* rb : A.produced) {
    if (rb->deviceOnly || !f.job.readback) continue;
    HIP_TRY(copyTileRows(rb, rb->stride, f.job, f.D.slot, f.st));
  }
  return GI_C_OK;
}

static int readBackAndWait(Frame& f, GiCRenderBuffer* colorRb)
{
  SceneDevice& D = f.D;
  HIP_TRY(hipMemcpyAsync(D.hCounters, D.dCounters.ptr, sizeof(Counters), hipMemcpyDeviceToHost, f.st));
  if (colorRb && !colorRb->deviceOnly && f.job.readback) HIP_TRY(copyTileRows(colorRb, 16, f.job, D.slot, f.st));
  HIP_TRY(hipStreamSynchronize(f.st));
  HIP_TRY(hipGetLastError());
  return GI_C_OK;
}

static void fillStats(const Frame& f, double tEnd)
{
  GiCRenderStats& S = f.D.stats; const Counters& c = *f.D.hCounters;
  S.renderMs = tEnd - f.tStart; S.samples = (uint64_t)f.pixels * f.rs.spp; S.iterations = f.iters; S.traceLaunches = f.traceLaunches;
  uint64_t* W = f.D.pathWalkStats;
  for (int k = 0; k < 18; k++) W[k] = 0u;
  if (f.served) {
    S.fusedPath = S.batches = S.poolSlots = 0u;
    S.segments = S.shadowRays = S.nodesVisited = S.trisTested = S.shadowNodesVisited = S.shadowTrisTested = 0u;
    return;
  }
  S.fusedPath = f.plan.fused ? 1u : 0u;
  S.segments = c.segments + f.skippedSegments; S.shadowRays = c.shadowRays; S.nodesVisited = c.nodesVisited; S.trisTested = c.trisTested;
  S.shadowNodesVisited = c.shadowNodesVisited; S.shadowTrisTested = c.shadowTrisTested;
  W[0] = c.phaseTrips; W[17] = c.walkFewLaneSteps;
  for (int k = 0; k < 8; k++) { W[1 + k] = c.walkStepTrips[k]; W[9 + k] = c.walkStepLanes[k]; }
}

extern "C" int giCDebugMissRect(const float* bounds, const GiCCameraDesc* camera, const GiCRenderSettings* settings, uint32_t width, uint32_t height, uint32_t* out)
{
  if (!bounds || !camera || !settings || !out || width == 0u || height == 0u) { setError("giCDebugMissRect: bad arguments"); return GI_C_ERROR; }
  FrameUniforms U{};
  cameraUniforms(*camera, width, height, U);
  U.flags = samplingFlags(*settings);
  const MissRect r = computeMissRect(bounds, bounds + 3, U, width, height);
  out[0] = r.x0; out[1] = r.y0; out[2] = r.x1; out[3] = r.y1;
  return GI_C_OK;
}

static void chooseShadowOrder(GiCScene* s, const Counters& c)
{
  if (s->shadowOrder.load() >= 0) return;
  for (int m = 0; m < 2; m++) {
    s->shadowOrderRays[m] += c.shadowOrderRays[m];
    for (int k = 0; k < 16; k++) s->shadowOrderSteps[m] += c.shadowOrderSteps[m][k].v;
  }
  constexpr uint64_t ENOUGH = 1u << 16;
  if (s->shadowOrderRays[0] < ENOUGH || s->shadowOrderRays[1] < ENOUGH) return;
  s->shadowOrder = (double)s->shadowOrderSteps[1] * (double)s->shadowOrderRays[0] < (double)s->shadowOrderSteps[0] * (double)s->shadowOrderRays[1] ? 1 : 0;
  if (getenv("GATLING_BUILD_TIMING")) {
    fprintf(stderr, "[gatling_gi] shadow walks: near-to-far %.3f node visits per ray (%llu rays), slot order %.3f (%llu rays) -> %s\n",
            (double)s->shadowOrderSteps[0] / (double)s->shadowOrderRays[0], (unsigned long long)s->shadowOrderRays[0],
            (double)s->shadowOrderSteps[1] / (double)s->shadowOrderRays[1], (unsigned long long)s->shadowOrderRays[1],
            s->shadowOrder.load() ? "slot order" : "near-to-far");
  }
}

static void printPhaseStats(const GiCScene* s, const Counters& c)
{
  if (!s->countTraversal || !optionValue("phase_stats", 0)) return;
  if (c.phaseTrips) {
    const double tot = (double)(c.phaseCycles[0] + c.phaseCycles[1] + c.phaseCycles[2] + c.phaseCycles[3]);
    static const char* names[4] = {"regen", "trace", "shade", "shadow+finish"};
    for (int k = 0; k < 4; k++) {
      fprintf(stderr, "[gatling_gi] k_path phase %-14s %5.1f %% of wave cycles, %5.1f of 64 lanes busy per trip\n", names[k],
              100.0 * (double)c.phaseCycles[k] / tot, (double)c.phaseLanes[k] / (double)c.phaseTrips);
    }
    fprintf(stderr, "[gatling_gi] k_path trips %llu, %.0f cycles per trip and wave\n", (unsigned long long)c.phaseTrips, tot / (double)c.phaseTrips);
    unsigned long long steps = 0ull;
    for (int k = 0; k < 8; k++) steps += c.walkStepTrips[k];
    for (int k = 0; k < 8 && c.walkStepTrips[k]; k++) {
      fprintf(stderr, "[gatling_gi] k_path walk step %d%s reached by %5.1f %% of the trips (%4.1f %% of all wave steps), %5.2f of 64 lanes walking\n", k,
              k == 7 ? "+" : " ", 100.0 * (double)c.walkStepTrips[k] / (double)c.phaseTrips, 100.0 * (double)c.walkStepTrips[k] / (double)steps,
              (double)c.walkStepLanes[k] / (double)c.walkStepTrips[k]);
    }
  }
  if (c.dynStats[0]) {
    const unsigned long long* d = c.dynStats; const double st = (double)d[0];
    fprintf(stderr, "[gatling_gi] k_trace_dyn<closest> %llu wave steps: per step %.1f lanes hold a ray, %.1f run the node test, %.1f wait for the triangle "
                    "ring; %.3f batches per step of %.1f pairs; "
                    "a refill every %.2f steps, %.1f lanes each\n",
            d[0], (double)d[1] / st, (double)d[2] / st, (double)d[3] / st, (double)d[4] / st, d[4] ? (double)d[5] / (double)d[4] : 0.0,
            d[6] ? st / (double)d[6] : 0.0, d[6] ? (double)d[7] / (double)d[6] : 0.0);
  }
}


struct LookaheadPlan { bool serve = false; uint32_t calls = 0; LookaheadKey key{}; };

static long lookaheadOption(const GiCScene* s)
{
  const long o = optionSet("lookahead") ? optionValue("lookahead", -1) : -1;
  return o >= 0 ? o : (long)s->optLookahead;
}

static LookaheadPlan planLookahead(Frame& f, const BoundAovs& A)
{
  Lookahead& L = f.D.lookahead;
  const GiCRenderSettings& rs = f.rs;
  LookaheadPlan la;
  const uint64_t N = (uint64_t)std::max(0L, lookaheadOption(f.s));
  if (N < 2u || !rs.progressiveAccumulation || A.nee || A.bounces || A.clock) { L.drop(); return la; }
  memset(&la.key, 0, sizeof(la.key));
  la.key.U = f.U; la.key.view = f.view; la.key.generation = f.s->generation;
  la.key.U.sampleOffset = 0u; la.key.U.sampleOffsetF = 0.0f; la.key.U.invTotalSampleCount = 0.0f;
  const bool continues = L.valid && (uint64_t)f.U.sampleOffset == (uint64_t)L.firstOffset + (uint64_t)L.served * rs.spp
                         && memcmp(&la.key.U, &L.key.U, sizeof(FrameUniforms)) == 0 && memcmp(&la.key.view, &L.key.view, sizeof(SceneView)) == 0
                         && la.key.generation == L.key.generation;
// ... 286 lines not shown
```

### gatling_amd/csrc/gi_shading.h

```cpp
#pragma once

#include "gi_queues.h"
#include "gi_texture.h"

namespace gi {

__device__ __forceinline__ uint32_t payload_medium_idx(uint32_t bitfield, uint32_t stackSize)
{
  const uint32_t idx = (bitfield & 0x0f000000u) >> 24, mx = stackSize > 1u ? stackSize : 1u;
  return idx < mx ? idx : mx;
}
__device__ __forceinline__ void payload_increment_walk(uint32_t& bitfield)
{
  uint32_t b = bitfield & 0x00fff000u;
  b = (b + 1u) < 0x00fff000u ? (b + 1u) : 0x00fff000u;
  bitfield &= ~0x00fff000u;
  bitfield |= b;
}

__device__ __forceinline__ void nee_aov_record_px(const PathState& st, uint32_t pixelLocal, uint32_t sampleLocal, bool shadowed)
{
  const unsigned long long order = (unsigned long long)(st.neeSampleBase + sampleLocal) + 1ull;
  atomicMax(&st.neeKey[pixelLocal], (order << 1) | (shadowed ? 1ull : 0ull));
}
// ... 271 lines not shown
}
__device__ inline GgxOut ggx_sample_xy(V3 l1, float ax, float ay, float x0, float x1)
{
  GgxOut o; o.valid = false; o.pdf = 0.0f; o.g2OverG1 = 0.0f; o.kh = 0.0f; o.l2 = v3(0.0f, 0.0f, 0.0f);
  V3 vh = normalize(v3(ax * l1.x, ay * l1.y, l1.z));
  float lensq = vh.x * vh.x + vh.y * vh.y;
  V3 T1 = lensq > 0.0f ? v3(-vh.y, vh.x, 0.0f) * (1.0f / gi_sqrt(lensq)) : v3(1.0f, 0.0f, 0.0f);
  V3 T2 = cross(vh, T1);
  float r = gi_sqrt(x0);
  float s, c; gi_sincos2pi(x1, &s, &c);
  float t1 = r * c, t2 = r * s;
  float sm = 0.5f * (1.0f + vh.z);
  t2 = (1.0f - sm) * gi_sqrt(fmax2(0.0f, 1.0f - t1 * t1)) + sm * t2;
  V3 nh = (T1 * t1 + T2 * t2) + vh * gi_sqrt(fmax2(0.0f, (1.0f - t1 * t1) - t2 * t2));
  V3 h = normalize(v3(ax * nh.x, ay * nh.y, fmax2(0.0f, nh.z)));
  float kh = dot(l1, h);
  V3 l2 = h * (2.0f * kh) - l1;
  if (!(l2.z > 0.0f) || !(kh > 0.0f)) return o;
  float nk1 = l1.z, nk2 = l2.z;
  float D = ggx_d_xy(ax, ay, h);
  float L1 = ggx_lambda_xy(ax, ay, l1), L2 = ggx_lambda_xy(ax, ay, l2);
  float G1 = 2.0f * nk1 / (nk1 + L1);
  float G2 = 2.0f * nk1 * nk2 / (nk2 * L1 + nk1 * L2);
  o.l2 = l2; o.kh = kh; o.pdf = G1 * D / (4.0f * nk1); o.g2OverG1 = G2 / G1; o.valid = true;
  return o;
}
__device__ inline void ggx_eval_xy(V3 l1, V3 l2, float ax, float ay, float& fcos, float& pdf, float& kh)
{
  fcos = 0.0f; pdf = 0.0f; kh = 0.0f;
  if (!(l1.z > 0.0f) || !(l2.z > 0.0f)) return;
  V3 h = normalize(l1 + l2);
  kh = dot(l1, h);
  float nk1 = l1.z, nk2 = l2.z;
  float D = ggx_d_xy(ax, ay, h);
  float L1 = ggx_lambda_xy(ax, ay, l1), L2 = ggx_lambda_xy(ax, ay, l2);
  float G1 = 2.0f * nk1 / (nk1 + L1);
  float G2 = 2.0f * nk1 * nk2 / (nk2 * L1 + nk1 * L2);
  fcos = D * G2 / (4.0f * nk1);
  pdf = G1 * D / (4.0f * nk1);
}
__device__ __forceinline__ void opbr_anisotropy(float alpha, float a, float& ax, float& ay)
{
  ax = alpha; ay = alpha;
  if (!(a > 0.0f)) return;
  const float inv = 1.0f - fmin2(a, 1.0f);
  ax = fmax2(alpha * gi_sqrt(2.0f / (1.0f + inv * inv)), 0.001f); ay = fmax2(inv * ax, 0.001f);
}
__device__ __forceinline__ GgxOut ggx_sample2(V3 l1, float ax, float ay, float x0, float x1)
{ return ax == ay ? ggx_sample(l1, ax, x0, x1) : ggx_sample_xy(l1, ax, ay, x0, x1); }
__device__ __forceinline__ void ggx_eval2(V3 l1, V3 l2, float ax, float ay, float& fcos, float& pdf, float& kh)
{ if (ax == ay) ggx_eval(l1, l2, ax, fcos, pdf, kh); else ggx_eval_xy(l1, l2, ax, ay, fcos, pdf, kh); }

__device__ __forceinline__ float relative_eta(const ShState& st, float materialEta)
{
  const bool outside = st.frontFace || st.thinWalled;
  float e1 = st.ior1 == 0.0f ? (outside ? 1.0f : -1.0f) : st.ior1;
  float e2 = st.ior2 == 0.0f ? (outside ? -1.0f : 1.0f) : st.ior2;
  if (e1 < 0.0f) e1 = materialEta;
  if (e2 < 0.0f) e2 = materialEta;
  return e2 / e1;
}
struct UpsParams { V3 albedo, F0; float alpha, coat, coatAlpha; };
__device__ __forceinline__ UpsParams ups_params(const MaterialRec* m, const ShState& st)
{
  UpsParams u;
  u.albedo = v3(m->p[MP_ALBEDO], m->p[MP_ALBEDO + 1], m->p[MP_ALBEDO + 2]);
  u.F0 = v3(m->p[MP_F0], m->p[MP_F0 + 1], m->p[MP_F0 + 2]);
  u.alpha = m->p[MP_ALPHA]; u.coat = m->p[MP_COAT]; u.coatAlpha = m->p[MP_COAT_ALPHA];
  if (st.texMask & ((1u << TEX_BASE_COLOR) | (1u << TEX_ROUGHNESS) | (1u << TEX_METALLIC))) {
    const V3 dc = (st.texMask & (1u << TEX_BASE_COLOR)) ? st.texBaseColor : v3(m->p[0], m->p[1], m->p[2]);
    const float r = (st.texMask & (1u << TEX_ROUGHNESS)) ? st.texRoughness : m->p[11];
    u.alpha = fmax2(r * r, 0.001f);
    if (m->p[6] != 0.0f) { u.F0 = v3(m->p[7], m->p[8], m->p[9]); u.albedo = dc; }
    else {
      const float ior = m->p[16], metal = (st.texMask & (1u << TEX_METALLIC)) ? st.texMetallic : m->p[10];
      const float q = (1.0f - ior) / (1.0f + ior), f0 = q * q;
      u.F0 = v3(f0, f0, f0) * (1.0f - metal) + dc * metal;
      u.albedo = dc * (1.0f - metal);
    }
  }
  return u;
}

struct BsdfSample { V3 k2, overPdf; float pdf; uint32_t event; };
struct BsdfEval { V3 diffuse, glossy; float pdf; };

__device__ __forceinline__ float fresnel_dielectric(float c, float eta)
{
  float sin2t = (1.0f - c * c) / (eta * eta);
  if (!(sin2t < 1.0f)) return 1.0f;
  float ct = gi_sqrt(1.0f - sin2t);
  float rs = (c - eta * ct) / (c + eta * ct);
  float rp = (eta * c - ct) / (eta * c + ct);
  return 0.5f * (rs * rs + rp * rp);
}
__device__ __forceinline__ V3 schlick_f82(V3 F0, V3 tint, float c)
{
  const float w5 = 0.462664366f, K = 17.6513846f;
  V3 one = v3(1.0f, 1.0f, 1.0f);
  V3 fb = F0 + (one - F0) * w5;
  V3 a = (fb * (one - tint)) * K;
  float m = 1.0f - c; m = fmin2(fmax2(m, 0.0f), 1.0f);
  float m2 = m * m, m5 = m2 * m2 * m, m6 = m5 * m;
  V3 f = (F0 + (one - F0) * m5) - a * (c * m6);
  return v3(fmin2(fmax2(f.x, 0.0f), 1.0f), fmin2(fmax2(f.y, 0.0f), 1.0f), fmin2(fmax2(f.z, 0.0f), 1.0f));
}
__device__ __forceinline__ float opbr_effective_roughness(float r, float cr, float coat)
{
  float c4 = (cr * cr) * (cr * cr), r4 = (r * r) * (r * r);
  float ra = gi_sqrt(gi_sqrt(fmin2(1.0f, 2.0f * c4 + r4)));
  return ra * coat + r * (1.0f - coat);
}
__device__ __forceinline__ V3 opbr_base_darkening(V3 baseColor, float sw, float metalness, float coat, float coatF0, float cior, float coatDarkening)
{
  const float w = coat * coatDarkening;
  if (w == 0.0f) return v3(1.0f, 1.0f, 1.0f);
  const float K = 1.0f - (1.0f - coatF0) / (cior * cior);
  const V3 Eb = (baseColor * sw) * metalness + baseColor * (1.0f - metalness);
  const float n = 1.0f - K;
  const V3 bd = v3(n / (1.0f - Eb.x * K), n / (1.0f - Eb.y * K), n / (1.0f - Eb.z * K));
  return bd * w + v3(1.0f, 1.0f, 1.0f) * (1.0f - w);
}
__device__ __forceinline__ V3 opbr_emission_factor(float coat, V3 coatColor, float coatF0, float c)
{
  if (coat == 0.0f) return v3(1.0f, 1.0f, 1.0f);
  const float f = (1.0f - coatF0) * (1.0f - schlick_w(c));
  return (coatColor * f) * coat + v3(1.0f, 1.0f, 1.0f) * (1.0f - coat);
}
__device__ __forceinline__ float eon_albedo_fit(float mu, float r)
{
  const float mc = 1.0f - mu;
  const float G = mc * (0.0571085289f + mc * (0.491881867f + mc * (-0.332181442f + mc * 0.0714429953f)));
  return (1.0f + r * G) / (1.0f + 0.28779343f * r);
}
__device__ inline V3 eon_pi_f(V3 rho, float r, V3 l1, V3 l2)
{
  const float mi = l1.z, mo = l2.z;
  const float s = l1.x * l2.x + l1.y * l2.y;
  const float sOverT = s > 0.0f ? s / fmax2(mi, mo) : s;
  const float AF = 1.0f / (1.0f + 0.28779343f * r);
  const float ss = AF * (1.0f + r * sOverT);
  const float EFo = eon_albedo_fit(mo, r), EFi = eon_albedo_fit(mi, r);
  const float avgEF = AF * (1.0f + 0.07248828f * r);
  const float ms = (fmax2(1e-7f, 1.0f - EFo) * fmax2(1e-7f, 1.0f - EFi)) / fmax2(1e-7f, 1.0f - avgEF);
  const V3 rr = rho * rho;
  const V3 rhoMs = v3((rr.x * avgEF) / (1.0f - rho.x * (1.0f - avgEF)), (rr.y * avgEF) / (1.0f - rho.y * (1.0f - avgEF)),
      (rr.z * avgEF) / (1.0f - rho.z * (1.0f - avgEF)));
  return rho * ss + rhoMs * ms;
}
struct OpbrParams { V3 albedo, metalTint, specColor, transTint, coatTint, baseColor, ssColor, fuzzColor;
    float metalness, alpha, alphaY, coat, coatAlpha, coatAlphaY, coatF0, eta, tw, specWeight, baseWeight, diffRough, ssWeight, ssAniso, fuzzWeight, fuzzAlpha,
    filmWeight, filmNm, filmIor, coatRotC, coatRotS; bool thinWalled, ssVolume, coatRot; };
__device__ __forceinline__ V3 coat_turn_local(const OpbrParams& o, V3 l)
{ return v3(l.x * o.coatRotC + l.y * o.coatRotS, l.y * o.coatRotC - l.x * o.coatRotS, l.z); }
__device__ __forceinline__ V3 coat_turn_world(const OpbrParams& o, V3 l)
{ return v3(l.x * o.coatRotC - l.y * o.coatRotS, l.x * o.coatRotS + l.y * o.coatRotC, l.z); }
__device__ __forceinline__ void spec_turn_frame(const MaterialRec* m, ShState& st)
{
  const float c = m->sss[8], s = m->sss[9];
  const V3 tu = st.tangentU * c + st.tangentV * s, tv = st.tangentV * c - st.tangentU * s;
  st.tangentU = tu; st.tangentV = tv;
}
__device__ __forceinline__ OpbrParams opbr_params(const MaterialRec* m, const ShState& st)
{
  OpbrParams o; const float* p = m->p;
  o.albedo = v3(p[MP_ALBEDO], p[MP_ALBEDO + 1], p[MP_ALBEDO + 2]);
  o.baseColor = v3(p[0], p[1], p[2]); o.baseWeight = p[17]; o.diffRough = p[27]; const uint32_t feat = (uint32_t)p[MP_FEATURES];
// ... 318 lines not shown
__device__ __forceinline__ OpbrBaseParams opbr_base_params(const MaterialRec* m)
{
  OpbrBaseParams o; const float* p = m->p;
  o.albedo = v3(p[MP_ALBEDO], p[MP_ALBEDO + 1], p[MP_ALBEDO + 2]);
  o.baseColor = v3(p[0], p[1], p[2]); o.baseWeight = p[17]; o.diffRough = p[27];
  o.metalTint = v3(p[MP_F0], p[MP_F0 + 1], p[MP_F0 + 2]);
  o.specColor = v3(p[7], p[8], p[9]);
  o.specWeight = p[18]; o.metalness = p[10];
  o.alpha = p[MP_ALPHA]; o.eta = p[MP_ETA];
  return o;
}
struct OpbrBaseCtx { V3 l1; float nk1, eta, Fd; bool have; };
__device__ __forceinline__ OpbrBaseCtx opbr_base_ctx(const MaterialRec* m, const ShState& st, V3 k1)
{
  OpbrBaseCtx c; c.l1 = to_local(st, k1); c.nk1 = fmax2(c.l1.z, 1e-4f); c.l1.z = c.nk1;
  c.eta = relative_eta(st, m->p[MP_ETA]); c.Fd = fresnel_dielectric(c.nk1, c.eta); c.have = true;
  return c;
}
__device__ inline void opbr_base_sample(const MaterialRec* m, const ShState& st, V3 k1, float x0, float x1, float x2, BsdfSample& out,
    const OpbrBaseCtx* ctx = nullptr)
{
  const OpbrBaseParams o = opbr_base_params(m);
  V3 l1 = ctx ? ctx->l1 : to_local(st, k1);
  const float nk1 = ctx ? ctx->nk1 : fmax2(l1.z, 1e-4f); l1.z = nk1;
  float z = x2;
  float eta = 0.0f, Fd = 0.0f;
  uint32_t lobe = 1u;
  if (!(z < o.metalness)) {
    z = (z - o.metalness) / (1.0f - o.metalness);
    eta = ctx ? ctx->eta : relative_eta(st, o.eta);
    Fd = ctx ? ctx->Fd : fresnel_dielectric(nk1, eta);
    lobe = 2u;
    if (!(z < Fd)) lobe = 4u;
  }
  if (lobe == 4u) {
    const float pBase = (1.0f - o.metalness) * (1.0f - Fd);
    const V3 l = gi_sample_hemisphere(x0, x1);
    const V3 k2 = to_world(st, l);
    if (!(l.z > 0.0f) || !(dot(k2, st.geomNormal) > 0.0f)) return;
    out.k2 = k2; out.pdf = pBase * (l.z / GI_PI);
    out.overPdf = (o.diffRough > 0.0f) ? eon_pi_f(o.baseColor, o.diffRough, l1, l) * o.baseWeight : o.albedo;
    out.event = EV_DIFFUSE | EV_REFLECTION;
    return;
  }
  const GgxOut g = ggx_sample(l1, o.alpha, x0, x1);
  const V3 k2 = to_world(st, g.l2);
  if (!g.valid || !(dot(k2, st.geomNormal) > 0.0f)) return;
  out.k2 = k2; out.event = EV_GLOSSY | EV_REFLECTION;
  if (lobe == 1u) {
    const V3 F = schlick_f82(o.albedo, o.metalTint, g.kh) * o.specWeight;
    out.pdf = o.metalness * g.pdf; out.overPdf = F * g.g2OverG1;
  } else {
    const float Fh = fresnel_dielectric(g.kh, eta);
    out.pdf = ((1.0f - o.metalness) * Fd) * g.pdf;
    out.overPdf = o.specColor * ((Fh / Fd) * g.g2OverG1);
  }
}
__device__ inline void opbr_base_evaluate(const MaterialRec* m, const ShState& st, V3 k1, V3 k2, BsdfEval& out, const OpbrBaseCtx* ctx = nullptr)
{
  const OpbrBaseParams o = opbr_base_params(m);
  V3 l1 = ctx ? ctx->l1 : to_local(st, k1); const V3 l2 = to_local(st, k2);
  const float nk1 = ctx ? ctx->nk1 : fmax2(l1.z, 1e-4f); l1.z = nk1;
  const float eta = ctx ? ctx->eta : relative_eta(st, o.eta);
  const float Fd = ctx ? ctx->Fd : fresnel_dielectric(nk1, eta);
  float fs, ps, khs; ggx_eval(l1, l2, o.alpha, fs, ps, khs);
  const float Fdh = fresnel_dielectric(khs, eta);
  const float cd = l2.z / GI_PI;
  const float diel = 1.0f - o.metalness;
  V3 gl = v3(0.0f, 0.0f, 0.0f);
  if (o.metalness != 0.0f) { const V3 Fm = schlick_f82(o.albedo, o.metalTint, khs) * o.specWeight; gl = gl + (Fm * fs) * o.metalness; }
  gl = gl + (o.specColor * (Fdh * fs)) * diel;
  out.glossy = gl;
  const V3 rho = (o.diffRough > 0.0f && l2.z > 0.0f) ? eon_pi_f(o.baseColor, o.diffRough, l1, l2) * o.baseWeight : o.albedo;
  out.diffuse = rho * ((cd * diel) * (1.0f - Fd));
  out.pdf = 0.0f + (o.metalness * ps + diel * (Fd * ps + (1.0f - Fd) * cd));
}

__device__ __forceinline__ V3 diffuse_class_color(const MaterialRec* m, const ShState& st)
{
  return (st.texMask & (1u << TEX_BASE_COLOR)) ? st.texBaseColor : v3(m->p[0], m->p[1], m->p[2]);
}

constexpr uint32_t KLASS_DYNAMIC = 0xffffffffu;
template <uint32_t KLASS>
__device__ inline void bsdf_sample(const MaterialRec* m, const ShState& st, V3 k1, float x0, float x1, float x2, BsdfSample& out)
{
  out.event = EV_ABSORB; out.pdf = 0.0f; out.overPdf = v3(0.0f, 0.0f, 0.0f); out.k2 = v3(0.0f, 0.0f, 0.0f);
  const uint32_t klass = (KLASS == KLASS_DYNAMIC) ? m->klass : KLASS;
  if (klass == 0u) {
    V3 l = gi_sample_hemisphere(x0, x1);
    V3 k2 = to_world(st, l);
    if (!(l.z > 0.0f) || !(dot(k2, st.geomNormal) > 0.0f)) return;
    out.k2 = k2; out.pdf = l.z / GI_PI; out.overPdf = diffuse_class_color(m, st); out.event = EV_DIFFUSE | EV_REFLECTION;
    return;
  }
  if (klass == 1u) {
    UpsParams u = ups_params(m, st);
    V3 l1 = to_local(st, k1);
    float nk1 = fmax2(l1.z, 1e-4f); l1.z = nk1;
    float z = x2;
    float Fc = u.coat * (0.04f + 0.96f * schlick_w(nk1));
    V3 Fs = v3(0.0f, 0.0f, 0.0f); float ps = 0.0f;
    uint32_t lobe = 0u;
    if (!(z < Fc)) {
      z = (z - Fc) / (1.0f - Fc);
      Fs = schlick3(u.F0, nk1);
      ps = fmax2(Fs.x, fmax2(Fs.y, Fs.z));
      lobe = (z < ps) ? 1u : 2u;
    }
    if (lobe != 2u) {
      GgxOut g = ggx_sample(l1, lobe == 0u ? u.coatAlpha : u.alpha, x0, x1);
      V3 k2 = to_world(st, g.l2);
      if (!g.valid || !(dot(k2, st.geomNormal) > 0.0f)) return;
      out.k2 = k2; out.event = EV_GLOSSY | EV_REFLECTION;
      if (lobe == 0u) {
        float Fh = u.coat * (0.04f + 0.96f * schlick_w(g.kh));
        float w = (Fh / Fc) * g.g2OverG1;
        out.pdf = Fc * g.pdf; out.overPdf = v3(w, w, w);
      } else {
        V3 Fh = schlick3(u.F0, g.kh);
        out.pdf = (1.0f - Fc) * ps * g.pdf; out.overPdf = Fh * (g.g2OverG1 / ps);
      }
      return;
    }
    V3 l = gi_sample_hemisphere(x0, x1);
    V3 k2 = to_world(st, l);
    if (!(l.z > 0.0f) || !(dot(k2, st.geomNormal) > 0.0f)) return;
    out.k2 = k2; out.pdf = (1.0f - Fc) * (1.0f - ps) * (l.z / GI_PI);
    out.overPdf = (u.albedo * (v3(1.0f, 1.0f, 1.0f) - Fs)) * (1.0f / (1.0f - ps));
    out.event = EV_DIFFUSE | EV_REFLECTION;
    return;
  }
  if (klass == 2u) { opbr_sample(m, st, k1, x0, x1, x2, out); return; }
  if (klass == SHADE_CLASS_OPBR_BASE) { opbr_base_sample(m, st, k1, x0, x1, x2, out); return; }
}

template <uint32_t KLASS>
__device__ inline void bsdf_evaluate(const MaterialRec* m, const ShState& st, V3 k1, V3 k2, BsdfEval& out)
{
  out.diffuse = v3(0.0f, 0.0f, 0.0f); out.glossy = v3(0.0f, 0.0f, 0.0f); out.pdf = 0.0f;
  float nk2 = dot(st.normal, k2);
  if (!(nk2 > 0.0f)) return;
  const uint32_t klass = (KLASS == KLASS_DYNAMIC) ? m->klass : KLASS;
  if (klass == 0u) {
    float c = nk2 / GI_PI;
    out.diffuse = diffuse_class_color(m, st) * c; out.pdf = c;
    return;
  }
  if (klass == 1u) {
    UpsParams u = ups_params(m, st);
    V3 l1 = to_local(st, k1), l2 = to_local(st, k2);
    float nk1 = fmax2(l1.z, 1e-4f); l1.z = nk1;
    float Fc = u.coat * (0.04f + 0.96f * schlick_w(nk1));
    V3 Fs = schlick3(u.F0, nk1);
    float ps = fmax2(Fs.x, fmax2(Fs.y, Fs.z));
    float fc, pc, khc; ggx_eval(l1, l2, u.coatAlpha, fc, pc, khc);
    float fs, pss, khs; ggx_eval(l1, l2, u.alpha, fs, pss, khs);
    float Fch = u.coat * (0.04f + 0.96f * schlick_w(khc));
    V3 Fsh = schlick3(u.F0, khs);
    float cd = l2.z / GI_PI;
    out.glossy = v3(Fch * fc, Fch * fc, Fch * fc) + (Fsh * fs) * (1.0f - Fc);
    out.diffuse = (u.albedo * (v3(1.0f, 1.0f, 1.0f) - Fs)) * (cd * (1.0f - Fc));
    out.pdf = Fc * pc + (1.0f - Fc) * (ps * pss + (1.0f - ps) * cd);
    return;
  }
  if (klass == 2u) { opbr_evaluate(m, st, k1, k2, out); return; }
  if (klass == SHADE_CLASS_OPBR_BASE) { opbr_base_evaluate(m, st, k1, k2, out); return; }
}

__device__ inline void sample_light(const SceneView& sc, const FrameUniforms& U, float k0, float k1, float k2, float k3, V3 surfacePos,
                                    V3& dirToLight, float& dist, V3& power, float& invPdf, uint32_t& dsPacked)
{
  const float sel = k0 * (float)U.totalLightCount;
  if (sel <= (float)U.sphereCount) {
    uint32_t idx = (uint32_t)(k1 * (float)U.sphereCount);
    const uint32_t last = U.sphereCount - 1u; if (idx > last) idx = last;
    V3 pos = v3(0.0f, 0.0f, 0.0f), em = pos, radius = pos; float area = 0.0f; dsPacked = 0u;
    if (idx < U.sphereCount) { const SphereLightRec l = sc.sphereLights[idx]; pos = v3(l.pos); em = v3(l.em); radius = v3(l.radius); area = l.area;
        dsPacked = l.ds; }
    V3 samplePos = pos + gi_sample_sphere(k2, k3, radius);
    V3 dir = samplePos - surfacePos;
    dist = length(dir);
    dirToLight = gi_safe_div(dir, dist);
    V3 ln = normalize(samplePos - pos);
    float cosTheta = fmax2(0.0f, dot(-dirToLight, ln));
    invPdf = gi_safe_div((area > 0.0f) ? (area * cosTheta) : 1.0f, dist * dist);
    power = em * U.lightIntensityMultiplier;
  } else if (sel <= (float)(U.sphereCount + U.distantCount)) {
    uint32_t idx = (uint32_t)(k1 * (float)U.distantCount);
    const uint32_t last = U.distantCount - 1u; if (idx > last) idx = last;
    const DistantLightRec l = sc.distantLights[idx];
    dist = 100000.0f; dirToLight = -v3(l.dir);
    power = v3(l.em) * U.lightIntensityMultiplier; invPdf = l.invPdf; dsPacked = l.ds;
// ... 45 lines not shown
```

### gatling_amd/csrc/gi_stages.h

```cpp
#pragma once

#include "gi_shading.h"

namespace gi {

__device__ __forceinline__ void make_camera_ray_at(const FrameUniforms& U, uint32_t px, uint32_t py, uint32_t pixelIndex, uint32_t sampleIndex, V3& origin,
    V3& dir, float& tMin, float& tMax, uint32_t& rng)
{
  rng = gi_hash_init(pixelIndex * (sampleIndex + 1u));
  float r0 = gi_next1f(rng), r1 = gi_next1f(rng);
  float sox = 0.5f, soy = 0.5f;
  if (U.flags & FLAG_JITTER) {
    if (U.flags & FLAG_FIS) { float gx, gy; gi_fis_gauss(r0, r1, gx, gy); sox = 0.5f + gx; soy = 0.5f + gy; }
    else { sox = r0; soy = r1; }
  }
  V3 camRight = v3(U.camRight), camUp = v3(U.camUp), camPos = v3(U.camPos);
  V3 P = (v3(U.L) + (camRight * ((float)px + sox)) * U.WX) + (camUp * ((float)py + soy)) * U.HY;
  origin = camPos;
  dir = normalize(P - origin);
  if ((U.flags & FLAG_DOF) && U.lensRadius > 0.0f) {
    float z0 = gi_next1f(rng), z1 = gi_next1f(rng);
    V3 focal = origin + dir * U.focusDistance;
    V3 ap = gi_sample_hemisphere(z0, z1);
    origin = origin + camRight * (ap.x * U.lensRadius);
    origin = origin + camUp * (ap.y * U.lensRadius);
    dir = normalize(focal - origin);
  }
  if (dir.x == 0.0f) dir.x += GI_FLT_MIN;
  if (dir.y == 0.0f) dir.y += GI_FLT_MIN;
  if (dir.z == 0.0f) dir.z += GI_FLT_MIN;
  tMin = 0.0f; tMax = GI_FLT_MAX;
  if (U.flags & FLAG_CLIP) {
    float cosCone = fmax2(1e-5f, dot(dir, v3(U.camFwd)));
    tMin = U.clipNear / cosCone; tMax = U.clipFar / cosCone;
  }
}

__device__ __forceinline__ void make_camera_ray(const FrameUniforms& U, uint32_t pixelIndex, uint32_t sampleIndex, V3& origin, V3& dir, float& tMin,
    float& tMax, uint32_t& rng)
{
  make_camera_ray_at(U, pixelIndex % U.imageWidth, pixelIndex / U.imageWidth, pixelIndex, sampleIndex, origin, dir, tMin, tMax, rng);
}

__device__ __forceinline__ V3 finish_sample(const FrameUniforms& U, V3 rad)
{
  const float mv = fmax2(rad.x, fmax2(rad.y, rad.z));
  if (mv > U.maxSampleValue) rad = rad * (U.maxSampleValue / mv);
  return v3(fmax2(0.0f, rad.x), fmax2(0.0f, rad.y), fmax2(0.0f, rad.z));
}

struct ShadeIO {
  V3 throughput, radiance; uint32_t bitfield, rng;
  bool cont, shadow, shadowFirst;
  V3 no, k2; float tMaxNext;
  V3 sdir, nee; float ld; uint32_t rngShadow;
};
template <uint32_t KLASS, bool TEXTURED, bool VOLUME, bool NEE, bool PACKED = false>
__device__ __forceinline__ void shade_segment(const FrameUniforms& U, const SceneView& sc, float* M , const F4& h,
    const F4& rd, ShadeIO& io)
{
  static_assert(KLASS != SHADE_CLASS_OPBR_BASE || (!TEXTURED && !VOLUME),
      "the BASE variant exists for untextured materials in renders without a medium stack (launchShade sends the others through the full kernel)");
  V3 throughput = io.throughput, radiance = io.radiance; uint32_t bitfield = io.bitfield, rng = io.rng;
  bool cont = false, shadow = false, shadowFirst = false; uint32_t rngShadow = 0u;
  V3 no = v3(0.0f, 0.0f, 0.0f), k2 = no, sdir = no, nee = no; float ld = 0.0f, tMaxNext = GI_FLT_MAX;
  const uint32_t bounce = bitfield & 0x00000fffu;

  const V3 rayDir = v3(rd.x, rd.y, rd.z);
  const uint32_t stackSize = VOLUME ? (U.mediumStackSize < MAX_MEDIUM_STACK ? U.mediumStackSize : MAX_MEDIUM_STACK) : 0u;
  uint32_t mediumIdx = payload_medium_idx(bitfield, stackSize);
  if (VOLUME && f2u(h.w) == VOLUME_MISS) {
    const float* m = M + (mediumIdx - 1u) * MEDIUM_FLOATS;
    const float* wp = M + stackSize * MEDIUM_FLOATS;
    const float distance = h.x * U.metersPerSceneUnit;
    const V3 sigS = v3(m[2], m[3], m[4]), sigT = v3(m[5], m[6], m[7]);
    const V3 tr = v3(gi_expf(sigT.x * -distance), gi_expf(sigT.y * -distance), gi_expf(sigT.z * -distance));
    const V3 density = sigT * tr;
    const float pdf = dot(v3(wp[0], wp[1], wp[2]), density);
    throughput = throughput * ((sigS * tr) / pdf);
    no = v3(h.y, h.z, rd.w) + rayDir * distance;
    k2 = rayDir;
    bitfield |= 0x40000000u;
    payload_increment_walk(bitfield);
  } else {
  ShState ss;
  setup_shading_state<PACKED>(sc, f2u(h.w), h.y, h.z, rayDir, ss);
  const MaterialRec* mat = &sc.materials[ss.material];
  if (TEXTURED && (mat->flags & MAT_FLAG_TEXTURED)) resolve_material_textures(sc, mat, rayDir, ss);
  if ((KLASS == 2u || (KLASS == KLASS_DYNAMIC && mat->klass == 2u)) && ((uint32_t)mat->p[MP_FEATURES] & MATF_SPEC_ROTATION)) spec_turn_frame(mat, ss);
  const bool isDoubleSided = (ss.meshFlags & 2u) != 0u;
  float prevMediumIor = 1.0f, nextMediumIor = 1.0f;
  if (mediumIdx > 0u) {
    const float distance = h.x * U.metersPerSceneUnit;
    if (!VOLUME) {
      if (((KLASS == KLASS_DYNAMIC) ? mat->klass : KLASS) == 2u
          || KLASS == SHADE_CLASS_OPBR_BASE) throughput = throughput * v3(gi_expf(-mat->p[MP_SIGMA_A] * distance), gi_expf(-mat->p[MP_SIGMA_A + 1] * distance),
          gi_expf(-mat->p[MP_SIGMA_A + 2] * distance));
    } else {
      const float* m = M + (mediumIdx - 1u) * MEDIUM_FLOATS;
      prevMediumIor = m[0];
      if (mediumIdx > 1u) nextMediumIor = M[(mediumIdx - 2u) * MEDIUM_FLOATS];
      throughput = throughput * v3(gi_expf(-m[5] * distance), gi_expf(-m[6] * distance), gi_expf(-m[7] * distance));
    }
  }
  const bool thinWalled = ((KLASS == KLASS_DYNAMIC) ? mat->klass : KLASS) == 2u && ((uint32_t)mat->p[MP_FEATURES] & MATF_THIN_WALLED) != 0u;
  ss.thinWalled = thinWalled;
  ss.sssVolume = VOLUME;
  if (VOLUME) { ss.ior1 = (ss.frontFace || thinWalled) ? prevMediumIor : -1.0f; ss.ior2 = (ss.frontFace || thinWalled) ? -1.0f : nextMediumIor; }
  V3 em = (ss.texMask & (1u << TEX_EMISSION)) ? ss.texEmission : v3(mat->p[3], mat->p[4], mat->p[5]);
  if (em.x != 0.0f || em.y != 0.0f || em.z != 0.0f) {
    if (ss.frontFace || !isDoubleSided) {
      const float c = dot(-rayDir, ss.normal);
      if (c > 0.0f) {
        if (((KLASS == KLASS_DYNAMIC) ? mat->klass : KLASS) == 2u)
          em = em * opbr_emission_factor(mat->p[12], v3(mat->p[19], mat->p[20], mat->p[21]), mat->p[MP_COAT_F0], c);
        radiance = radiance + throughput * (em * U.exposureScale);
      }
    }
  }
  const float x0 = gi_next1f(rng), x1 = gi_next1f(rng), x2 = gi_next1f(rng); (void)gi_next1f(rng);
  BsdfSample bs;
  OpbrBaseCtx baseCtx; baseCtx.have = false;
  if constexpr (KLASS == SHADE_CLASS_OPBR_BASE && NEE) {
    baseCtx = opbr_base_ctx(mat, ss, -rayDir);
    bs.event = EV_ABSORB; bs.pdf = 0.0f; bs.overPdf = v3(0.0f, 0.0f, 0.0f); bs.k2 = v3(0.0f, 0.0f, 0.0f);
    opbr_base_sample(mat, ss, -rayDir, x0, x1, x2, bs, &baseCtx);
  } else bsdf_sample<KLASS>(mat, ss, -rayDir, x0, x1, x2, bs);
  throughput = throughput * bs.overPdf;
  k2 = bs.k2;
  const bool isTransmission = (bs.event & EV_TRANSMISSION) != 0u;
  if (NEE && (bs.event & (EV_DIFFUSE | EV_GLOSSY))) {
    const float k0 = gi_next1f(rng), k1 = gi_next1f(rng), kk2 = gi_next1f(rng), k3 = gi_next1f(rng);
    V3 dirToLight, lightPower; float lightDist, invPdf; uint32_t ds;
    sample_light(sc, U, k0, k1, kk2, k3, ss.position, dirToLight, lightDist, lightPower, invPdf, ds);
    if ((lightDist > 0.0f) && dot(dirToLight, ss.geomNormal) > 0.0f) {
      BsdfEval ev;
      if constexpr (KLASS == SHADE_CLASS_OPBR_BASE && NEE) {
        ev.diffuse = v3(0.0f, 0.0f, 0.0f); ev.glossy = v3(0.0f, 0.0f, 0.0f); ev.pdf = 0.0f;
        if (dot(ss.normal, dirToLight) > 0.0f) opbr_base_evaluate(mat, ss, -rayDir, dirToLight, ev, &baseCtx);
      } else bsdf_evaluate<KLASS>(mat, ss, -rayDir, dirToLight, ev);
      if (ev.pdf > 0.0f) {
        const float dmul = gi_half_to_float(ds & 0xffffu), smul = gi_half_to_float(ds >> 16);
        const V3 weight = throughput * (lightPower * invPdf);
        nee = nee + (weight * ev.diffuse) * dmul;
        nee = nee + (weight * ev.glossy) * smul;
      }
    }
    const V3 toLight = dirToLight * lightDist;
    ld = length(toLight);
    sdir = gi_safe_div(toLight, ld);
    shadow = gi_luminance(nee) > 1e-6f && ld > 1e-9f;
    rngShadow = rng;
  }
  shadowFirst = bounce == 0u;
  if (KLASS != SHADE_CLASS_OPBR_BASE && !thinWalled && isTransmission) {
    uint32_t newIdx = mediumIdx;
    if (VOLUME) {
      if (ss.frontFace) {
        newIdx = mediumIdx + 1u;
        if (newIdx <= stackSize) {
          float* m = M + (newIdx - 1u) * MEDIUM_FLOATS;
          if (KLASS == 2u) {
            const float depth = mat->p[28];
            const V3 sigS = (depth > 0.0f) ? v3(mat->p[29] / depth, mat->p[30] / depth, mat->p[31] / depth) : v3(0.0f, 0.0f, 0.0f);
            const V3 sigT = v3(mat->p[MP_SIGMA_A], mat->p[MP_SIGMA_A + 1], mat->p[MP_SIGMA_A + 2]) + sigS;
            m[0] = mat->p[MP_ETA]; m[1] = mat->p[47]; m[2] = sigS.x; m[3] = sigS.y; m[4] = sigS.z; m[5] = sigT.x; m[6] = sigT.y; m[7] = sigT.z;
            if (bs.event & EV_SUBSURFACE) { m[1] = mat->p[59]; m[2] = mat->sss[0]; m[3] = mat->sss[1]; m[4] = mat->sss[2]; m[5] = mat->sss[3];
                m[6] = mat->sss[4]; m[7] = mat->sss[5]; }
          } else { m[0] = 1.0f; m[1] = 0.0f; m[2] = 0.0f; m[3] = 0.0f; m[4] = 0.0f; m[5] = 0.0f; m[6] = 0.0f; m[7] = 0.0f; }
        }
      } else if (mediumIdx > 0u) newIdx = mediumIdx - 1u;
    } else newIdx = 1u - mediumIdx;
    bitfield &= ~0x00fff000u;
    bitfield = (bitfield & ~0x0f000000u) | ((newIdx << 24) & 0x0f000000u);
  }
  if (bs.event == EV_ABSORB) bitfield |= 0x80000000u;
  const V3 gn = ss.geomNormal * (isTransmission ? -1.0f : 1.0f);
  no = gi_offset_ray_origin(ss.position, gn);
  }
  if (length(throughput) < 1e-9f) bitfield |= 0x80000000u;
  if (bounce > U.rrBounceOffset) {
    const float k = gi_next1f(rng);
    const float mt = fmax2(throughput.x, fmax2(throughput.y, throughput.z));
    const float p = fmin2(mt, U.rrInvMinTermProb);
    if (k > p) bitfield |= 0x80000000u; else throughput = throughput / p;
  }
  if (VOLUME && (bitfield & 0x40000000u)) {
    const float x0 = gi_next1f(rng), x1 = gi_next1f(rng);
    const float g = M[(mediumIdx - 1u) * MEDIUM_FLOATS + 1u];
    float cosTheta;
    if (fabsf(g) < 1e-3f) cosTheta = 1.0f - 2.0f * x0;
    else { const float sq = (1.0f - g * g) / ((1.0f - g) + (2.0f * g) * x0); cosTheta = ((1.0f + g * g) - sq * sq) / (2.0f * g); }
    const float sinTheta = gi_sqrt(fmax2(0.0f, 1.0f - cosTheta * cosTheta));
    float sp, cp; gi_sincos2pi(x1, &sp, &cp);
    V3 t, b; gi_orthonormal_basis(k2, t, b);
    k2 = ((t * sinTheta) * cp + (b * sinTheta) * sp) + k2 * cosTheta;
    bitfield &= ~0x40000000u;
  }
  bitfield++;
  cont = ((bitfield & 0x00000fffu) < U.maxBounces) && !(bitfield & 0x80000000u);
  if (VOLUME && cont) {
    const uint32_t idx2 = payload_medium_idx(bitfield, stackSize);
    if (idx2 > 0u) {
      const float* m = M + (idx2 - 1u) * MEDIUM_FLOATS;
      float* wp = M + stackSize * MEDIUM_FLOATS;
      V3 wpdf = v3(1.0f, 1.0f, 1.0f);
      const uint32_t walkLength = (bitfield & 0x00fff000u) >> 12;
      const V3 sigS = v3(m[2], m[3], m[4]), sigT = v3(m[5], m[6], m[7]);
      if ((sigS.x > 0.0f || sigS.y > 0.0f || sigS.z > 0.0f) && walkLength <= U.maxVolumeWalkLength) {
// ... 71 lines not shown
```

### gatling_amd/csrc/gi_types.h

```cpp
#pragma once

#include <stdint.h>

namespace gi {

struct Node8 {
  float p[3];
  uint8_t e[3];
  uint8_t imask;
  uint32_t childBase;
  uint32_t triBase;
  uint8_t meta[8];
  uint8_t qlo[3][8];
  uint8_t qhi[3][8];
};
static_assert(sizeof(Node8) == 80, "Node8 must be 80 bytes");

struct TriRec {
  float v0[3];
  float e1[3];
  float e2[3];
  uint32_t origId;
  uint32_t instance;
  uint32_t matFlags;
// ... 124 lines not shown
  const TriRec* tris;
  const InstanceRec* instances;
  const FVertex* verts;
  const F4* triGeomNormal;
  const TriShade* triShade; uint32_t shadePacked;
  const MaterialRec* materials;
  const SphereLightRec* sphereLights;
  const DistantLightRec* distantLights;
  const RectLightRec* rectLights;
  const DiskLightRec* diskLights;
  const LightFrame* rectFrames; const LightFrame* diskFrames;
  const int32_t* triFaceId;
  uint32_t nodeCount;
  uint32_t triCount;
  uint32_t bvhDepth;
  uint32_t hasCutouts;
  const TextureRec* textures;
  const MeshRec* meshes;
  const float* sceneData;
  uint32_t domeTexture;
  uint32_t domeCameraVisible;
  float domeRotation[4];
  float domeEmission[3];
  float background[3];
  float cameraPosition[3];
  float frame;
  uint32_t mediumStackSize;
  const Node8* tlasNodes; const uint32_t* tlasItems;
  const Node8* blasNodes; const BlasTri* blasTris;
  const InstTrav* instTrav;
  const uint32_t* flatOfOrig;
  uint32_t twoLevel;
};


struct AovTargets {
  F4* normal; F4* barycentrics; F4* texcoords; F4* opacity; F4* tangents; F4* bitangents; F4* thinWalled; F4* doubleSided; F4* albedo;
  float* depth; int32_t* objectId; int32_t* faceId; int32_t* instanceId;
  float clear[17][4];
};

struct alignas(64) Slot {
  F4 thr;
  F4 rad;
  F4 id;
  F4 pad;
};
static_assert(sizeof(Slot) == 64, "Slot must be 64 bytes");

constexpr uint32_t MEDIUM_FLOATS = 8, MAX_MEDIUM_STACK = 15;
constexpr uint32_t VOLUME_MISS = 0xfffffffeu;
struct PathState {
  Slot* slots; float* media; uint32_t mediaStride;
  unsigned long long* neeKey; uint32_t neeSampleBase; F4* bouncesAov;
  uint32_t* pathSegments;
};

constexpr uint32_t MAT_CLASS_COUNT = 4, SHADE_CLASS_OPBR_BASE = 3;
enum : uint32_t { Q_TRACE_A = 0, Q_TRACE_B = 1, Q_REGEN_A = 2, Q_REGEN_B = 3, Q_SHADOW = 4, Q_HIT = 5, Q_COUNT = Q_HIT + MAT_CLASS_COUNT };
constexpr uint32_t NSHARD = 8;
constexpr uint32_t NCURSOR = 8;
struct FreshRec { uint32_t rng, work; };
struct QueueSet {
  FreshRec* fresh[2];
  uint32_t* slot[Q_COUNT];
  F4* a[Q_COUNT];
  F4* b[Q_COUNT];
  F4* c[Q_COUNT];
  uint32_t cap;
};
struct alignas(128) PaddedCounter { uint32_t v; uint32_t pad[31]; };
struct Counters {
  PaddedCounter count[Q_COUNT][NSHARD];
  PaddedCounter workBase[2];
  PaddedCounter cursor[2][NCURSOR];
  unsigned long long segments, shadowRays, nodesVisited, trisTested, shadowNodesVisited, shadowTrisTested;
  unsigned long long shadowOrderRays[2];
  PaddedCounter shadowOrderSteps[2][16];
  uint32_t overflow;
  unsigned long long phaseCycles[4], phaseLanes[4], phaseTrips;
  unsigned long long walkStepLanes[8], walkStepTrips[8];
  unsigned long long dynStats[8];
  unsigned long long walkFewLaneSteps;
};

}
```

### include/gi_c.h

```cpp
#ifndef GATLING_GI_C_H
#define GATLING_GI_C_H

#include <stdint.h>
#include <stddef.h>

#ifdef __cplusplus
extern "C" {
#endif

#define GI_C_OK 0
#define GI_C_ERROR 1

#define GI_C_MAX_AOV_COMP_SIZE 16

typedef enum GiCAovId {
  GI_C_AOV_COLOR = 0, GI_C_AOV_NORMAL, GI_C_AOV_NEE, GI_C_AOV_BARYCENTRICS, GI_C_AOV_TEXCOORDS, GI_C_AOV_BOUNCES,
  GI_C_AOV_CLOCK_CYCLES, GI_C_AOV_OPACITY, GI_C_AOV_TANGENTS, GI_C_AOV_BITANGENTS, GI_C_AOV_THIN_WALLED,
  GI_C_AOV_OBJECT_ID, GI_C_AOV_DEPTH, GI_C_AOV_FACE_ID, GI_C_AOV_INSTANCE_ID, GI_C_AOV_DOUBLE_SIDED, GI_C_AOV_ALBEDO,
  GI_C_AOV_COUNT
} GiCAovId;

typedef enum GiCRenderBufferFormat { GI_C_FORMAT_INT32 = 0, GI_C_FORMAT_FLOAT32 = 1, GI_C_FORMAT_FLOAT32_VEC4 = 2 } GiCRenderBufferFormat;

typedef struct GiCScene GiCScene;
// ... 266 lines not shown
void giCDestroySphereLight(GiCScene* scene, GiCSphereLight* light);
void giCSetSphereLightPosition(GiCSphereLight* light, const float* position);
void giCSetSphereLightBaseEmission(GiCSphereLight* light, const float* rgb);
void giCSetSphereLightRadius(GiCSphereLight* light, float radiusX, float radiusY, float radiusZ);
void giCSetSphereLightDiffuseSpecular(GiCSphereLight* light, float diffuse, float specular);

GiCDistantLight* giCCreateDistantLight(GiCScene* scene);
void giCDestroyDistantLight(GiCScene* scene, GiCDistantLight* light);
void giCSetDistantLightDirection(GiCDistantLight* light, const float* direction);
void giCSetDistantLightBaseEmission(GiCDistantLight* light, const float* rgb);
void giCSetDistantLightAngle(GiCDistantLight* light, float angle);
void giCSetDistantLightDiffuseSpecular(GiCDistantLight* light, float diffuse, float specular);

GiCRectLight* giCCreateRectLight(GiCScene* scene);
void giCDestroyRectLight(GiCScene* scene, GiCRectLight* light);
void giCSetRectLightOrigin(GiCRectLight* light, const float* origin);
void giCSetRectLightTangents(GiCRectLight* light, const float* t0, const float* t1);
void giCSetRectLightBaseEmission(GiCRectLight* light, const float* rgb);
void giCSetRectLightDimensions(GiCRectLight* light, float width, float height);
void giCSetRectLightDiffuseSpecular(GiCRectLight* light, float diffuse, float specular);

GiCDiskLight* giCCreateDiskLight(GiCScene* scene);
void giCDestroyDiskLight(GiCScene* scene, GiCDiskLight* light);
void giCSetDiskLightOrigin(GiCDiskLight* light, const float* origin);
void giCSetDiskLightTangents(GiCDiskLight* light, const float* t0, const float* t1);
void giCSetDiskLightBaseEmission(GiCDiskLight* light, const float* rgb);
void giCSetDiskLightRadius(GiCDiskLight* light, float radiusX, float radiusY);
void giCSetDiskLightDiffuseSpecular(GiCDiskLight* light, float diffuse, float specular);

GiCDomeLight* giCCreateDomeLight(GiCScene* scene, const char* filePath);
void giCSetDomeLightTexture(GiCDomeLight* light, GiCTexture* texture);
void giCDestroyDomeLight(GiCDomeLight* light);
void giCSetDomeLightRotation(GiCDomeLight* light, const float* quat);
void giCSetDomeLightBaseEmission(GiCDomeLight* light, const float* rgb);
void giCSetDomeLightDiffuseSpecular(GiCDomeLight* light, float diffuse, float specular);

GiCRenderBuffer* giCCreateRenderBuffer(uint32_t width, uint32_t height, int32_t format );
void giCDestroyRenderBuffer(GiCRenderBuffer* renderBuffer);
void* giCGetRenderBufferMem(GiCRenderBuffer* renderBuffer);

void* giCGetRenderBufferDeviceMem(GiCRenderBuffer* renderBuffer);
void giCSetRenderBufferDeviceOnly(GiCRenderBuffer* renderBuffer, int32_t deviceOnly);
int giCGetRenderStats(const GiCScene* scene, GiCRenderStats* out);
#define GI_C_SCENE_OPTION_COUNT_TRAVERSAL 1
#define GI_C_SCENE_OPTION_KERNEL_TIMERS 2
#define GI_C_SCENE_OPTION_POOL_SLOTS 3
#define GI_C_SCENE_OPTION_SAMPLE_BUFFER_MB 4
#define GI_C_SCENE_OPTION_TRACE_DYNAMIC 5
#define GI_C_SCENE_OPTION_TWO_LEVEL 6
#define GI_C_SCENE_OPTION_FUSED_PATH 7
#define GI_C_SCENE_OPTION_DEVICES 8
#define GI_C_SCENE_OPTION_BVH_BUILD 9
#define GI_C_SCENE_OPTION_SAMPLE_LOOKAHEAD 10
#define GI_C_SCENE_OPTION_VISIBILITY_UPDATES 11
#define GI_C_SCENE_OPTION_VERTEX_UPDATES 12
#define GI_C_SCENE_OPTION_TOPOLOGY_UPDATES 13
#define GI_C_SCENE_OPTION_RESYNC_REFITS 14
int giCGetLookaheadStats(const GiCScene* scene, GiCLookaheadStats* out);
int giCSetSceneOption(GiCScene* scene, int32_t option, int32_t value);
int giCTraceRays(GiCScene* scene, uint32_t count, const float* origins , const float* dirs ,
                 float tMin, float tMax, float* outTUV , int32_t* outInstPrim );

int giCDebugEvalBsdf(const GiCMaterialDesc* desc, uint32_t count, const float* in, float* out);
int giCDebugShadeClass(const GiCMaterialDesc* desc);
int64_t giCDebugCheckSqrt(uint32_t first, uint64_t count);
int giCDebugTexRuntime(const float* rgba, uint32_t width, uint32_t height, uint32_t depth, uint32_t count, const float* queries, float* out);
int giCDebugValidateBvh(const float* triVerts, uint32_t triCount, uint32_t* outNodeCount, uint32_t* outMaxDepth);
int giCDebugValidatePartitionedBvh(const float* triVerts, uint32_t triCount, uint32_t partCount, uint32_t* outNodeCount, uint32_t* outMaxDepth);
int giCDebugRefitBvh(const float* triVertsA, const float* triVertsB, uint32_t triCount, uint32_t* outNodeCount, uint32_t* outMaxDepth);
int giCDebugSceneRefitCheck(const GiCScene* scene, uint32_t deviceIndex, uint32_t* outNodes);
int giCDebugValidateSceneBvh(const GiCScene* scene, uint32_t deviceIndex, uint32_t* outNodeCount, uint32_t* outMaxDepth, int32_t* outBuiltOnDevice,
                             uint64_t* outDigest);

int32_t giCDebugEditDirtyFlags(int32_t edit, int32_t built);
int giCDebugSceneUpdateCounts(const GiCScene* scene, uint64_t* outCounts );
int giCDebugSceneVisibilityUpdateCount(const GiCScene* scene, uint64_t* outCount);
int giCDebugSceneVertexUpdateCount(const GiCScene* scene, uint64_t* outCount);
int giCDebugSceneTopologyUpdateCount(const GiCScene* scene, uint64_t* outCount);
int giCDebugSceneResyncCount(const GiCScene* scene, uint64_t* outCount);
int giCDebugGatherShade(const GiCVertex* vertices, uint32_t vertexCount, const GiCFace* faces, uint32_t faceCount);
int giCDebugSceneShadeCheck(const GiCScene* scene, uint32_t deviceIndex, uint32_t* outRecords);
int giCDebugSceneClassState(const GiCScene* scene, uint32_t* out );
int giCDebugPathWalkStats(const GiCScene* scene, uint64_t* out );
int giCDebugMissRect(const float* bounds , const GiCCameraDesc* camera, const GiCRenderSettings* settings, uint32_t width, uint32_t height,
                     uint32_t* out );

#ifdef __cplusplus
}
#endif
#endif
```

Measured before the change: 12640 Msamples/s.

## Park glossy-lobe shading lanes in LDS lot to reduce wave divergence

```diff
diff --git a/gatling_amd/capi.py b/gatling_amd/capi.py
--- a/gatling_amd/capi.py
+++ b/gatling_amd/capi.py
@@ -163,6 +163,8 @@
     ("giCDebugSceneResyncCount", C.c_int, [_P, C.POINTER(C.c_uint64)]), ("giCDebugGatherShade", C.c_int, [_P, _U, _P, _U]),
     ("giCDebugSceneShadeCheck", C.c_int, [_P, _U, C.POINTER(C.c_uint32)]),
     ("giCDebugPathWalkStats", C.c_int, [_P, C.POINTER(C.c_uint64)]),
+    ("giCDebugPathLobeStats", C.c_int, [_P, C.POINTER(C.c_uint64)]),
+    ("giCDebugPathLot", C.c_int, [C.c_uint32, C.c_uint32, C.c_uint32, C.POINTER(C.c_uint32)]),
     ("giCDebugMissRect", C.c_int, [_FP, C.POINTER(GiCCameraDesc), C.POINTER(GiCRenderSettings), _U, _U, C.POINTER(C.c_uint32)]),
 ]
 
@@ -510,6 +512,13 @@
             raise GiError("giCDebugPathWalkStats failed")
         return {"phaseTrips": int(c[0]), "stepTrips": [int(v) for v in c[1:9]], "stepLanes": [int(v) for v in c[9:17]], "fewLaneSteps": int(c[17])}
 
+    def path_lobe_stats(self) -> dict:
+        c = (C.c_uint64 * 9)()
+        if self.L.giCDebugPathLobeStats(self.handle, c) != GI_C_OK:
+            raise GiError("giCDebugPathLobeStats failed")
+        keys = ("shaded", "glossy", "glossyTrips", "liteTrips", "fullTrips", "parked", "adopted", "reruns", "rerunHits")
+        return {k: int(v) for k, v in zip(keys, c)}
+
     def set_option(self, option: int, value: int):
         if self.L.giCSetSceneOption(self.handle, option, value) != GI_C_OK:
             raise GiError("giCSetSceneOption failed")
diff --git a/gatling_amd/csrc/gi_debug.cpp b/gatling_amd/csrc/gi_debug.cpp
--- a/gatling_amd/csrc/gi_debug.cpp
+++ b/gatling_amd/csrc/gi_debug.cpp
@@ -518,6 +518,23 @@
   return GI_C_OK;
 }
 
+extern "C" int giCDebugPathLobeStats(const GiCScene* scene, uint64_t* out)
+{
+  GiCScene* s = const_cast<GiCScene*>(scene);
+  if (!s || !out) { setError("giCDebugPathLobeStats: bad arguments"); return GI_C_ERROR; }
+  std::lock_guard<std::mutex> guard(s->mutex);
+  for (int k = 0; k < 9; k++) out[k] = s->pathLobeStats[k];
+  return GI_C_OK;
+}
+
+extern "C" int giCDebugPathLot(uint32_t bvhDepth, uint32_t nodeCount, uint32_t triCount, uint32_t* out)
+{
+  if (!out) { setError("giCDebugPathLot: bad arguments"); return GI_C_ERROR; }
+  const gi::PathLot lot = gi::pathLotPlacement(bvhDepth);
+  out[0] = lot.stack; out[1] = lot.row; out[2] = lot.capacity; out[3] = gi::traceLdsBytes(lot.stack, nodeCount, triCount);
+  return GI_C_OK;
+}
+
 extern "C" int giCDebugSceneClassState(const GiCScene* scene, uint32_t* out)
 {
   GiCScene* s = const_cast<GiCScene*>(scene);
diff --git a/gatling_amd/csrc/gi_host.h b/gatling_amd/csrc/gi_host.h
--- a/gatling_amd/csrc/gi_host.h
+++ b/gatling_amd/csrc/gi_host.h
@@ -239,6 +239,7 @@
   hipEvent_t evShade = nullptr, evShadow = nullptr;
   GiCRenderStats stats{};
   uint64_t pathWalkStats[18] = {};
+  uint64_t pathLobeStats[9] = {};
   std::vector<hipEvent_t> eventPool;
   template <typename Fn> void forEachPathBuffer(Fn&& fn)
   {
diff --git a/gatling_amd/csrc/gi_kernels.h b/gatling_amd/csrc/gi_kernels.h
--- a/gatling_amd/csrc/gi_kernels.h
+++ b/gatling_amd/csrc/gi_kernels.h
@@ -37,9 +37,17 @@
     bool volume , const FrameUniforms& U, const SceneView& sc, const PathState& st, const QueueSet& qs, Counters* cnt, uint32_t par);
 
 bool pathKernelSupports(const SceneView& sc);
-int launchPath(hipStream_t s, uint32_t cuCount, uint32_t classMask, bool textured, bool count, uint32_t chunk, uint32_t walkCarry, const FrameUniforms& U,
-               const SceneView& sc, const PathState& st, Counters* cnt, F4* sampleBuf);
+int launchPath(hipStream_t s, uint32_t cuCount, uint32_t classMask, bool textured, bool count, uint32_t chunk, uint32_t walkCarry, uint32_t lobePark,
+               const FrameUniforms& U, const SceneView& sc, const PathState& st, Counters* cnt, F4* sampleBuf);
 constexpr long WALK_CARRY_DEFAULT = 8;
+constexpr long LOBE_PARK_DEFAULT = 8;
+struct PathLot { uint32_t stack, row, capacity; };
+inline PathLot pathLotPlacement(uint32_t bvhDepth)
+{
+  const uint32_t stack = bvhDepth <= 4u ? 4u : 8u;
+  const uint32_t row = bvhDepth < stack ? bvhDepth : stack;
+  return PathLot{stack, row, (stack - row) * 8u};
+}
 
 void launchAov(hipStream_t s, const FrameUniforms& U, const SceneView& sc, const AovTargets& A);
 void launchResolveNee(hipStream_t s, const FrameUniforms& U, const unsigned long long* key, F4* aov, uint32_t pixelCount);
diff --git a/gatling_amd/csrc/gi_kernels.hip b/gatling_amd/csrc/gi_kernels.hip
--- a/gatling_amd/csrc/gi_kernels.hip
+++ b/gatling_amd/csrc/gi_kernels.hip
@@ -31,6 +31,7 @@
                           cnt->shadowTrisTested = 0;
                       for (int k = 0; k < 4; k++) { cnt->phaseCycles[k] = 0; cnt->phaseLanes[k] = 0; } cnt->phaseTrips = 0;
                       for (int k = 0; k < 8; k++) { cnt->walkStepLanes[k] = 0; cnt->walkStepTrips[k] = 0; } cnt->walkFewLaneSteps = 0;
+                      for (int k = 0; k < 9; k++) cnt->lobeStats[k] = 0;
                           for (int k = 0; k < 8; k++) cnt->dynStats[k] = 0; }
   }
   for (; i < n; i += gridDim.x * blockDim.x) qs.slot[Q_REGEN_A][(i / per) * qs.cap + (i % per)] = i | REGEN_FRESH;
diff --git a/gatling_amd/csrc/gi_path.hip b/gatling_amd/csrc/gi_path.hip
--- a/gatling_amd/csrc/gi_path.hip
+++ b/gatling_amd/csrc/gi_path.hip
@@ -1,5 +1,6 @@
 
 #include <hip/hip_runtime.h>
+#include <cassert>
 
 #define GI_LEAN_SQRT 1
 #include "gi_device_math.h"
@@ -18,9 +19,12 @@
 constexpr int PATH_WAVES = 4;
 template <uint32_t KLASS, bool TEXTURED, bool NEE, bool CUTOUT, bool COUNT, uint32_t PATH_STACK>
 __global__ __launch_bounds__(TRACE_BLOCK) __attribute__((amdgpu_waves_per_eu(PATH_WAVES, 8))) void k_path(FrameUniforms U, SceneView sc, PathState st,
-    Counters* cnt, F4* __restrict__ sampleBuf, uint32_t ldsNodes, uint32_t ldsTris, uint32_t chunk, uint32_t walkCarry)
+    Counters* cnt, F4* __restrict__ sampleBuf, uint32_t ldsNodes, uint32_t ldsTris, uint32_t chunk, uint32_t walkCarry, uint32_t lobePark, uint32_t lotRow,
+    uint32_t lotCap)
 {
   constexpr bool CARRY = !NEE;
+  constexpr bool PARK = !NEE && (KLASS == 1u || (KLASS == KLASS_DYNAMIC && COUNT));
+  constexpr bool DEFER = PARK || COUNT;
   const StagedScene S = stage_scene<PATH_STACK>(sc, ldsNodes, ldsTris);
   __shared__ WaveTri s_wave[TRACE_BLOCK / 64];
   WaveTri& W = s_wave[threadIdx.x >> 6];
@@ -44,6 +48,14 @@
   unsigned long long pc[4] = {0ull, 0ull, 0ull, 0ull}, pl[4] = {0ull, 0ull, 0ull, 0ull}, trips = 0ull, tPrev = COUNT ? __builtin_readcyclecounter() : 0ull;
   uint32_t whLanes[8] = {0u, 0u, 0u, 0u, 0u, 0u, 0u, 0u}, whTrips[8] = {0u, 0u, 0u, 0u, 0u, 0u, 0u, 0u};
   uint32_t whFew = 0u;
+  uint32_t lobeN[9] = {0u, 0u, 0u, 0u, 0u, 0u, 0u, 0u, 0u};
+  const uint32_t lotFit = (PATH_STACK - (lotRow < PATH_STACK ? lotRow : PATH_STACK)) * 8u;
+  const uint32_t lotMax = PARK ? (lotCap < lotFit ? lotCap : lotFit) : 0u;
+  const uint32_t parkAt = PARK ? (lobePark < lotMax ? lobePark : lotMax) : 0u;
+  uint32_t lotCount = 0u;
+  auto lot_record = [&](uint32_t k) __attribute__((always_inline)) {
+    return (volatile GI_LDS gi_u4*)(GI_LDS gi_u4*)&S.stack[lotRow + (k >> 3)][(threadIdx.x & ~63u) + ((k & 7u) << 3)];
+  };
   auto phase = [&](int k,
       unsigned long long lanes) { if (COUNT) { const unsigned long long t = __builtin_readcyclecounter(); pc[k] += t - tPrev; tPrev = t; pl[k] += lanes; } };
   for (;;) {
@@ -103,7 +115,7 @@
       }
       preHead += take;
     }
-    if (!__ballot(alive)) break;
+    if (!__ballot(alive) && (!PARK || lotCount == 0u)) break;
     phase(0, nIdle); trips++;
 
     {
@@ -135,17 +147,36 @@
     const bool walked = CARRY ? alive && !tAlive : alive;
     bool ended = false;
     ShadeIO io; io.shadow = false; io.shadowFirst = false; io.cont = false;
+    if (DEFER) { io.lite = false; io.glossyLobe = false; io.deferred = false; }
     phase(1, (unsigned long long)__popcll(__ballot(walked)));
+    auto finish_path = [&]() __attribute__((always_inline)) {
+      const uint32_t bounces = bitfield & 0x00000fffu;
+      if (st.bouncesAov && U.batchFirstSample + rec / U.pixelCount == U.spp - 1u) {
+        const uint32_t maxB = U.maxBounces < 0x00000fffu ? U.maxBounces : 0x00000fffu;
+        const V3 c = gi_colormap_inferno((float)bounces / (float)maxB);
+        F4* dst = &st.bouncesAov[tile_to_image_pixel(U, rec % U.pixelCount)];
+        dst->x = c.x; dst->y = c.y; dst->z = c.z;
+      }
+      if (st.pathSegments) atomicAdd(&st.pathSegments[rec % U.pixelCount], bounces);
+      const V3 c = finish_sample(U, rad);
+      st4(&sampleBuf[rec], c.x, c.y, c.z, 0.0f);
+      alive = false;
+    };
+    bool shaded = false;
+    uint32_t nEarly = 0u;
     if (walked) {
       nSeg++;
       wave_ray_end(W, R);
       if (R.found) {
-        io.throughput = thr; io.radiance = rad; io.bitfield = bitfield; io.rng = rng;
-        const F4 h = F4{R.tBest, R.bestU, R.bestV, u2f(R.bestTri)}, rd = F4{rdv.x, rdv.y, rdv.z, 0.0f};
-        shade_segment<KLASS, TEXTURED, false, NEE>(U, sc, nullptr, h, rd, io);
-        thr = io.throughput; rad = io.radiance; bitfield = io.bitfield; rng = io.rng;
-        if (NEE && st.neeKey && io.shadowFirst && !io.shadow) nee_aov_record_px(st, rec % U.pixelCount, rec / U.pixelCount, false);
-        ended = !io.cont;
+        if constexpr (!PARK) {
+          io.throughput = thr; io.radiance = rad; io.bitfield = bitfield; io.rng = rng;
+          const F4 h = F4{R.tBest, R.bestU, R.bestV, u2f(R.bestTri)}, rd = F4{rdv.x, rdv.y, rdv.z, 0.0f};
+          shade_segment<KLASS, TEXTURED, false, NEE, false, DEFER>(U, sc, nullptr, h, rd, io);
+          thr = io.throughput; rad = io.radiance; bitfield = io.bitfield; rng = io.rng;
+          if (NEE && st.neeKey && io.shadowFirst && !io.shadow) nee_aov_record_px(st, rec % U.pixelCount, rec / U.pixelCount, false);
+          ended = !io.cont;
+          shaded = true;
+        }
       } else {
         rad = rad + thr * v3(U.background);
         if (st.neeKey && (bitfield & 0x00000fffu) == 0u) nee_aov_record_px(st, rec % U.pixelCount, rec / U.pixelCount, false);
@@ -153,7 +184,65 @@
         ended = true;
       }
     }
-    phase(2, (unsigned long long)__popcll(__ballot(walked && R.found)));
+    if constexpr (PARK) {
+      bool hit = walked && R.found;
+      auto shade_hit = [&]() __attribute__((always_inline)) {
+        io.throughput = thr; io.radiance = rad; io.bitfield = bitfield; io.rng = rng;
+        const F4 h = F4{R.tBest, R.bestU, R.bestV, u2f(R.bestTri)}, rd = F4{rdv.x, rdv.y, rdv.z, 0.0f};
+        shade_segment<KLASS, TEXTURED, false, NEE, false, DEFER>(U, sc, nullptr, h, rd, io);
+        if (io.deferred) return;
+        thr = io.throughput; rad = io.radiance; bitfield = io.bitfield; rng = io.rng;
+        ended = !io.cont;
+        shaded = true;
+        if (!ended) { ro = io.no; rdv = io.k2; tMin = 0.0f; tMax = io.tMaxNext; }
+      };
+      bool lite = lotCount < parkAt && !(exhausted && preTail == preHead) && __ballot(hit) != 0ull;
+      if (COUNT && parkAt) lobeN[lite ? 3 : 4]++;
+      for (;;) {
+        if (!lite && lotCount) {
+          nEarly += (uint32_t)__popcll(__ballot(ended));
+          if (ended) { finish_path(); ended = false; }
+          const unsigned long long freeLanes = __ballot(!alive);
+          const uint32_t nFree = (uint32_t)__popcll(freeLanes), nAdopt = nFree < lotCount ? nFree : lotCount;
+          const uint32_t rank = (uint32_t)__popcll(freeLanes & below);
+          __atomic_signal_fence(__ATOMIC_SEQ_CST);
+          if (!alive && rank < nAdopt) {
+            volatile GI_LDS gi_u4* p = lot_record(lotCount - nAdopt + rank);
+            const gi_u4 a = p[0], b = p[1], c = p[2], d = p[3];
+            thr = v3(u2f(a.x), u2f(a.y), u2f(a.z)); bitfield = a.w; rad = v3(u2f(b.x), u2f(b.y), u2f(b.z)); rng = b.w;
+            rdv = v3(u2f(c.x), u2f(c.y), u2f(c.z)); rec = c.w; R.tBest = u2f(d.x); R.bestU = u2f(d.y); R.bestV = u2f(d.z); R.bestTri = d.w;
+            alive = true; hit = true;
+          }
+          lotCount -= nAdopt;
+          if (COUNT) lobeN[6] += nAdopt;
+        }
+        io.lite = lite;
+        if (hit) shade_hit();
+        const unsigned long long deferred = lite ? __ballot(hit && io.deferred) : 0ull;
+        if (!deferred) break;
+        const uint32_t nDeferred = (uint32_t)__popcll(deferred);
+        if (lotCount + nDeferred <= lotMax) {
+          if (hit && io.deferred) {
+            volatile GI_LDS gi_u4* p = lot_record(lotCount + (uint32_t)__popcll(deferred & below));
+            p[0] = gi_u4{f2u(thr.x), f2u(thr.y), f2u(thr.z), bitfield}; p[1] = gi_u4{f2u(rad.x), f2u(rad.y), f2u(rad.z), rng};
+            const uint4 wh = wt_hit_get(W, lane);
+            p[2] = gi_u4{f2u(rdv.x), f2u(rdv.y), f2u(rdv.z), rec}; p[3] = gi_u4{wt_best_t(W, lane), wh.y, wh.z, wh.x};
+            alive = false;
+          }
+          __atomic_signal_fence(__ATOMIC_SEQ_CST);
+          lotCount += nDeferred;
+          if (COUNT) lobeN[5] += nDeferred;
+          break;
+        }
+        hit = hit && io.deferred; lite = false;
+        if (COUNT) { lobeN[7]++; lobeN[8] += nDeferred; }
+      }
+    }
+    if (COUNT) {
+      const unsigned long long glossy = __ballot(shaded && io.glossyLobe);
+      lobeN[0] += (uint32_t)__popcll(__ballot(shaded)); lobeN[1] += (uint32_t)__popcll(glossy); lobeN[2] += glossy ? 1u : 0u;
+    }
+    phase(2, (unsigned long long)__popcll(__ballot(PARK ? shaded : walked && R.found)));
 
     if (NEE) {
       bool sAlive = alive && io.shadow;
@@ -172,7 +261,8 @@
       }
     }
 
-    if (walked) {
+    if constexpr (PARK) { if (ended) finish_path(); }
+    else if (walked) {
       if (!ended) { ro = io.no; rdv = io.k2; tMin = 0.0f; tMax = io.tMaxNext; }
       else {
         const uint32_t bounces = bitfield & 0x00000fffu;
@@ -188,14 +278,15 @@
         alive = false;
       }
     }
-    phase(3, (unsigned long long)__popcll(__ballot(ended)));
+    phase(3, (unsigned long long)__popcll(__ballot(ended)) + nEarly);
   }
 
   if (COUNT
       && lane == 0u) { for (int k = 0; k < 4; k++) { atomicAdd(&cnt->phaseCycles[k], pc[k]); atomicAdd(&cnt->phaseLanes[k], pl[k]);
       } atomicAdd(&cnt->phaseTrips, trips);
       for (int k = 0; k < 8; k++) { atomicAdd(&cnt->walkStepLanes[k], (unsigned long long)whLanes[k]); atomicAdd(&cnt->walkStepTrips[k], (unsigned long long)whTrips[k]); }
-      atomicAdd(&cnt->walkFewLaneSteps, (unsigned long long)whFew); }
+      atomicAdd(&cnt->walkFewLaneSteps, (unsigned long long)whFew);
+      for (int k = 0; k < 9; k++) atomicAdd(&cnt->lobeStats[k], (unsigned long long)lobeN[k]); }
   unsigned long long a = nSeg, b = nShadow, c = tc.nodes, d = tc.tris, e = tcs.nodes, f = tcs.tris;
   for (int off = 32; off > 0; off >>= 1) {
     a += __shfl_down(a, off); b += __shfl_down(b, off);
@@ -216,7 +307,7 @@
          && !sc.shadePacked;
 }
 
-using PathKernel = void (*)(FrameUniforms, SceneView, PathState, Counters*, F4*, uint32_t, uint32_t, uint32_t, uint32_t);
+using PathKernel = void (*)(FrameUniforms, SceneView, PathState, Counters*, F4*, uint32_t, uint32_t, uint32_t, uint32_t, uint32_t, uint32_t, uint32_t);
 template <uint32_t STACK>
 static PathKernel pickPathKernel(uint32_t classMask, bool textured, bool nee, bool cutout, bool count)
 {
@@ -232,12 +323,14 @@
   }, nee);
 }
 
-int launchPath(hipStream_t s, uint32_t cuCount, uint32_t classMask, bool textured, bool count, uint32_t chunk, uint32_t walkCarry, const FrameUniforms& U,
-               const SceneView& sc, const PathState& st, Counters* cnt, F4* sampleBuf)
+int launchPath(hipStream_t s, uint32_t cuCount, uint32_t classMask, bool textured, bool count, uint32_t chunk, uint32_t walkCarry, uint32_t lobePark,
+               const FrameUniforms& U, const SceneView& sc, const PathState& st, Counters* cnt, F4* sampleBuf)
 {
   if (U.workTotal == 0u) return 0;
   const uint32_t ldsNodes = sc.nodeCount, ldsTris = sc.triCount;
-  const uint32_t stack = sc.bvhDepth <= 4u ? 4u : 8u;
+  const PathLot lot = pathLotPlacement(sc.bvhDepth);
+  const uint32_t stack = lot.stack;
+  assert(sc.bvhDepth <= stack && lot.row >= sc.bvhDepth && lot.row + (lot.capacity + 7u) / 8u <= stack);
   const uint32_t bytes = traceLdsBytes(stack, ldsNodes, ldsTris);
   const bool neeOn = (U.flags & FLAG_NEE) != 0u;
   PathKernel k = stack == 4u
@@ -256,7 +349,7 @@
   const uint64_t needed = (chunks + (TRACE_BLOCK / 64u) - 1u) / (TRACE_BLOCK / 64u);
   if (blocks > needed) blocks = needed;
   if (blocks == 0u) blocks = 1u;
-  hipLaunchKernelGGL(k, dim3((uint32_t)blocks), dim3(TRACE_BLOCK), bytes, s, U, sc, st, cnt, sampleBuf, ldsNodes, ldsTris, chunk, walkCarry);
+  hipLaunchKernelGGL(k, dim3((uint32_t)blocks), dim3(TRACE_BLOCK), bytes, s, U, sc, st, cnt, sampleBuf, ldsNodes, ldsTris, chunk, walkCarry, lobePark, lot.row, lot.capacity);
   return perCu;
 }
 
diff --git a/gatling_amd/csrc/gi_render.cpp b/gatling_amd/csrc/gi_render.cpp
--- a/gatling_amd/csrc/gi_render.cpp
+++ b/gatling_amd/csrc/gi_render.cpp
@@ -369,6 +369,7 @@
   long twoStreamDelay = 0;
   uint32_t dynRefill = 8u;
   uint32_t walkCarry = 0u;
+  uint32_t lobePark = 0u;
   int32_t shadowOrderNow = -1;
 };
 struct Frame {
@@ -433,6 +434,7 @@
   }
   Schedule sch;
   sch.walkCarry = s->countTraversal && !optionSet("walk_carry") ? 0u : (uint32_t)std::min(std::max(optionValue("walk_carry", WALK_CARRY_DEFAULT), 0L), 63L);
+  sch.lobePark = s->countTraversal && !optionSet("lobe_park") ? 0u : (uint32_t)std::min(std::max(optionValue("lobe_park", LOBE_PARK_DEFAULT), 0L), 64L);
   sch.dynRefill = traceDynRefill(s);
   sch.shadowOrderNow = optionSet("shadow_order") ? (int32_t)optionValue("shadow_order", -1) : s->shadowOrder.load();
   sch.twoStreamOk = rs.nextEventEstimation != 0 && rs.mediumStackSize == 0u && f.view.domeTexture == 0u && optionValue("two_stream", 1) != 0
@@ -470,7 +472,7 @@
   chunk = (uint32_t)std::min<uint64_t>(chunk, std::max<uint64_t>(64u, ((uint64_t)U.workTotal / (waves * 16u)) & ~63ull));
   f.tm.beginIteration(true);
   f.tm.timed(f.st, StageTimers::TRACE, [&] {
-    launchPath(f.st, (uint32_t)f.ctx.cuCount, s->classMask, s->classTextured != 0u, s->countTraversal, chunk, f.sch.walkCarry, U, f.view, f.ps,
+    launchPath(f.st, (uint32_t)f.ctx.cuCount, s->classMask, s->classTextured != 0u, s->countTraversal, chunk, f.sch.walkCarry, f.sch.lobePark, U, f.view, f.ps,
                D.dCounters.ptr, D.sampleBuf.ptr);
   });
   f.iters++; f.tm.totalIters++; f.traceLaunches++;
@@ -633,6 +635,7 @@
   S.renderMs = tEnd - f.tStart; S.samples = (uint64_t)f.pixels * f.rs.spp; S.iterations = f.iters; S.traceLaunches = f.traceLaunches;
   uint64_t* W = f.D.pathWalkStats;
   for (int k = 0; k < 18; k++) W[k] = 0u;
+  for (int k = 0; k < 9; k++) f.D.pathLobeStats[k] = 0u;
   if (f.served) {
     S.fusedPath = S.batches = S.poolSlots = 0u;
     S.segments = S.shadowRays = S.nodesVisited = S.trisTested = S.shadowNodesVisited = S.shadowTrisTested = 0u;
@@ -642,6 +645,7 @@
   S.segments = c.segments + f.skippedSegments; S.shadowRays = c.shadowRays; S.nodesVisited = c.nodesVisited; S.trisTested = c.trisTested;
   S.shadowNodesVisited = c.shadowNodesVisited; S.shadowTrisTested = c.shadowTrisTested;
   W[0] = c.phaseTrips; W[17] = c.walkFewLaneSteps;
+  for (int k = 0; k < 9; k++) f.D.pathLobeStats[k] = c.lobeStats[k];
   for (int k = 0; k < 8; k++) { W[1 + k] = c.walkStepTrips[k]; W[9 + k] = c.walkStepLanes[k]; }
 }
 
diff --git a/gatling_amd/csrc/gi_shading.h b/gatling_amd/csrc/gi_shading.h
--- a/gatling_amd/csrc/gi_shading.h
+++ b/gatling_amd/csrc/gi_shading.h
@@ -377,7 +377,9 @@
   return u;
 }
 
-struct BsdfSample { V3 k2, overPdf; float pdf; uint32_t event; };
+struct BsdfSample { V3 k2, overPdf; float pdf; uint32_t event;
+  bool glossyLobe, deferred;
+};
 struct BsdfEval { V3 diffuse, glossy; float pdf; };
 
 __device__ __forceinline__ float fresnel_dielectric(float c, float eta)
@@ -862,10 +864,11 @@
 }
 
 constexpr uint32_t KLASS_DYNAMIC = 0xffffffffu;
-template <uint32_t KLASS>
-__device__ inline void bsdf_sample(const MaterialRec* m, const ShState& st, V3 k1, float x0, float x1, float x2, BsdfSample& out)
+template <uint32_t KLASS, bool DEFER = false>
+__device__ inline void bsdf_sample(const MaterialRec* m, const ShState& st, V3 k1, float x0, float x1, float x2, BsdfSample& out, bool lite = false)
 {
   out.event = EV_ABSORB; out.pdf = 0.0f; out.overPdf = v3(0.0f, 0.0f, 0.0f); out.k2 = v3(0.0f, 0.0f, 0.0f);
+  if (DEFER) { out.glossyLobe = false; out.deferred = false; }
   const uint32_t klass = (KLASS == KLASS_DYNAMIC) ? m->klass : KLASS;
   if (klass == 0u) {
     V3 l = gi_sample_hemisphere(x0, x1);
@@ -889,6 +892,7 @@
       lobe = (z < ps) ? 1u : 2u;
     }
     if (lobe != 2u) {
+      if (DEFER) { out.glossyLobe = true; if (lite) { out.deferred = true; return; } }
       GgxOut g = ggx_sample(l1, lobe == 0u ? u.coatAlpha : u.alpha, x0, x1);
       V3 k2 = to_world(st, g.l2);
       if (!g.valid || !(dot(k2, st.geomNormal) > 0.0f)) return;
diff --git a/gatling_amd/csrc/gi_stages.h b/gatling_amd/csrc/gi_stages.h
--- a/gatling_amd/csrc/gi_stages.h
+++ b/gatling_amd/csrc/gi_stages.h
@@ -54,8 +54,9 @@
   bool cont, shadow, shadowFirst;
   V3 no, k2; float tMaxNext;
   V3 sdir, nee; float ld; uint32_t rngShadow;
+  bool lite, glossyLobe, deferred;
 };
-template <uint32_t KLASS, bool TEXTURED, bool VOLUME, bool NEE, bool PACKED = false>
+template <uint32_t KLASS, bool TEXTURED, bool VOLUME, bool NEE, bool PACKED = false, bool DEFER = false>
 __device__ __forceinline__ void shade_segment(const FrameUniforms& U, const SceneView& sc, float* M , const F4& h,
     const F4& rd, ShadeIO& io)
 {
@@ -65,6 +66,7 @@
   bool cont = false, shadow = false, shadowFirst = false; uint32_t rngShadow = 0u;
   V3 no = v3(0.0f, 0.0f, 0.0f), k2 = no, sdir = no, nee = no; float ld = 0.0f, tMaxNext = GI_FLT_MAX;
   const uint32_t bounce = bitfield & 0x00000fffu;
+  if constexpr (DEFER) { io.glossyLobe = false; io.deferred = false; }
 
   const V3 rayDir = v3(rd.x, rd.y, rd.z);
   const uint32_t stackSize = VOLUME ? (U.mediumStackSize < MAX_MEDIUM_STACK ? U.mediumStackSize : MAX_MEDIUM_STACK) : 0u;
@@ -125,6 +127,10 @@
     baseCtx = opbr_base_ctx(mat, ss, -rayDir);
     bs.event = EV_ABSORB; bs.pdf = 0.0f; bs.overPdf = v3(0.0f, 0.0f, 0.0f); bs.k2 = v3(0.0f, 0.0f, 0.0f);
     opbr_base_sample(mat, ss, -rayDir, x0, x1, x2, bs, &baseCtx);
+  } else if constexpr (DEFER) {
+    bsdf_sample<KLASS, true>(mat, ss, -rayDir, x0, x1, x2, bs, io.lite);
+    io.glossyLobe = bs.glossyLobe; io.deferred = bs.deferred;
+    if (bs.deferred) return;
   } else bsdf_sample<KLASS>(mat, ss, -rayDir, x0, x1, x2, bs);
   throughput = throughput * bs.overPdf;
   k2 = bs.k2;
diff --git a/gatling_amd/csrc/gi_types.h b/gatling_amd/csrc/gi_types.h
--- a/gatling_amd/csrc/gi_types.h
+++ b/gatling_amd/csrc/gi_types.h
@@ -230,6 +230,7 @@
   unsigned long long walkStepLanes[8], walkStepTrips[8];
   unsigned long long dynStats[8];
   unsigned long long walkFewLaneSteps;
+  unsigned long long lobeStats[9];
 };
 
 }
diff --git a/include/gi_c.h b/include/gi_c.h
--- a/include/gi_c.h
+++ b/include/gi_c.h
@@ -372,6 +372,8 @@
 int giCDebugSceneShadeCheck(const GiCScene* scene, uint32_t deviceIndex, uint32_t* outRecords);
 int giCDebugSceneClassState(const GiCScene* scene, uint32_t* out );
 int giCDebugPathWalkStats(const GiCScene* scene, uint64_t* out );
+int giCDebugPathLobeStats(const GiCScene* scene, uint64_t* out );
+int giCDebugPathLot(uint32_t bvhDepth, uint32_t nodeCount, uint32_t triCount, uint32_t* out );
 int giCDebugMissRect(const float* bounds , const GiCCameraDesc* camera, const GiCRenderSettings* settings, uint32_t width, uint32_t height,
                      uint32_t* out );
 
```

Result: faster. 13090 Msamples/s, median of 6 (+3.5%).
